# anenbergb/Co-DETR-TensorRT

Hardware: AMD Instinct MI355X
Metric: images/sec, Co-DINO Swin-L 1920x1280 fp16 (p50 ms/image alongside) (higher is better)
Workload: dtype f16

## Files before the change

__graft_entry__.py:

```python
import os
import subprocess
import sys

ROOT = os.path.dirname(os.path.abspath(__file__))
PKG_ROOT = os.path.join(ROOT, "co-detr-tensorrt_amd")
for _p in (ROOT, PKG_ROOT, os.path.join(ROOT, "oracle")):
    if _p not in sys.path:
        sys.path.insert(0, _p)


def _newer(target, sources):
    if not os.path.isfile(target):
        return True
    t = os.path.getmtime(target)
    return any(os.path.getmtime(s) > t for s in sources)


def build() -> None:
    csrc = os.path.join(PKG_ROOT, "csrc")
    so = os.path.join(PKG_ROOT, "codetr", "libcodetr_hip.so")
    srcs = [os.path.join(csrc, f) for f in os.listdir(csrc) if f.endswith((".hip", ".h", "Makefile"))]
    srcs += [os.path.join(ROOT, "include", h) for h in ("codetr_hip.h", "codetr_jpeg.h", "codetr_jpeg_dec.h", "codetr_assign.h", "codetr_wbf.h", "codetr_motion.h", "codetr_appearance.h", "codetr_redact.h")]
    if _newer(so, srcs):
        subprocess.check_call(["make", "-C", csrc, "-s", "-j4"])
    runner_dir = os.path.join(ROOT, "runner")
    runner = os.path.join(runner_dir, "codetr_runner")
    if _newer(runner, [os.path.join(runner_dir, f) for f in ("codetr_runner.cpp", "dispatch_gen.inc", "Makefile")]):
        subprocess.check_call(["make", "-C", runner_dir, "-s"])
    import msda_oracle

    msda_oracle.build()
    import codetr


def smoke() -> None:
    build()
    import smoke_impl

    smoke_impl.run()


if __name__ == "__main__":
    build()
    print("build ok")
    if len(sys.argv) > 1 and sys.argv[1] == "smoke":
        smoke()
        print("smoke ok")
```

co-detr-tensorrt_amd/codetr/_kernel_names.py:

```python
KERNEL_NAMES = (
    "add_kernel",
    "appearance_describe_kernel",
    "assign_kernel",
    "batched_nms_kernel",
    "cast_fp8_kernel",
    "cast_fp8mx_kernel",
    "conv_im2col_nchw_kernel",
    "conv_tokens_kernel",
    "decode_boxes_kernel",
    "decoder_layer_kernel",
    "draw_detections_kernel",
    "encoder_geometry_kernel",
    "ffn_fp8_kernel",
    "ffn_fused_kernel",
    "frames_to_rgb_kernel",
    "gather_rows_kernel",
    "gn_apply_kernel",
    "gn_finalize_kernel",
    "gn_partial_kernel",
    "im2col_tokens_kernel",
    "jpeg_encode_rows_kernel",
    "jpeg_gather_rows_kernel",
    "jpegdec_coefficients",
    "jpegdec_idct",
    "jpegdec_link_runs",
    "jpegdec_pixels",
    "jpegdec_sync_runs",
    "layernorm_fp8_kernel",
    "layernorm_fp8mx_kernel",
    "layernorm_kernel",
    "level_cums_kernel",
    "level_mask_kernel",
    "linear_256_fp8_kernel",
    "linear_256_kernel",
    "linear_kernel",
    "linear_pp_kernel",
    "linear_sk_kernel",
    "linear_xs_kernel",
    "maxpool_tokens_kernel",
    "mha_attention_kernel",
    "motion_finish_kernel",
    "motion_match_kernel",
    "motion_sim_fit_kernel",
    "motion_sim_pairs_kernel",
    "motion_thumb_kernel",
    "msda_backward_generic_kernel",
    "msda_backward_kernel",
    "msda_encoder_v4_kernel",
    "msda_fused_headmajor_kernel",
    "msda_op4_kernel",
    "msda_scalar_kernel",
    "msda_tiled_kernel",
    "pack_w2_kernel",
    "patch_im2col_k4_kernel",
    "postprocess_kernel",
    "postprocess_softnms_kernel",
    "preprocess_batch_kernel",
    "preprocess_kernel",
    "preprocess_tiles_kernel",
    "preprocess_views_kernel",
    "query_sine_embed_kernel",
    "redact_kernel",
    "row_max_kernel",
    "sigmoid_kernel",
    "sine_pos_kernel",
    "slice_merge_kernel",
    "splitk_reduce_kernel",
    "swin_mlp_kernel",
    "topk_kernel",
    "topk_reg_kernel",
    "track_kernel",
    "tta_merge_kernel",
    "valid_ratios_kernel",
    "wbf_merge_kernel",
    "window_attention_kernel",
)
```

co-detr-tensorrt_amd/codetr/export.py:

```python
import ctypes
import struct

import torch

from . import _cabi

MAGIC = b"CODETRPLAN\x00\x02"
import re

from ._kernel_names import KERNEL_NAMES

_OWN_DEMANGLED = re.compile(r"^(?:void )?\(anonymous namespace\)::(" + "|".join(KERNEL_NAMES) + r")\s*[<(]")
_OWN_MANGLED = re.compile(r"^_ZN12_GLOBAL__N_1(\d+)([A-Za-z_][A-Za-z0-9_]*)")


def is_own_kernel(name: str) -> bool:
    if _OWN_DEMANGLED.match(name):
        return True
    m = _OWN_MANGLED.match(name)
    return bool(m) and m.group(2)[:int(m.group(1))] in KERNEL_NAMES
KIND_INT, KIND_FLOAT, KIND_DEV, KIND_NULL, KIND_HOST, KIND_STREAM = 0, 1, 2, 3, 4, 5


def _hip():
    for name in ("libamdhip64.so", "libamdhip64.so.7", "libamdhip64.so.6"):
        try:
            return ctypes.CDLL(name)
        except OSError:
            continue
    raise RuntimeError("libamdhip64.so not found")


def _read_device(hip, addr, nbytes):
    buf = ctypes.create_string_buffer(nbytes)
    rc = hip.hipMemcpy(buf, ctypes.c_void_p(addr), ctypes.c_size_t(nbytes), 2)
    if rc != 0:
        raise RuntimeError(f"hipMemcpy D2H of {nbytes} bytes at {addr:#x} failed with {rc}")
    return buf.raw


def _segments(device):
    segs = []
    for s in torch.cuda.memory_snapshot():
        if s.get("device", 0) != device.index:
            continue
        blocks, addr = [], s["address"]
        for b in s["blocks"]:
            a = b.get("address", addr)
            blocks.append((a, b["size"], b["state"]))
            addr = a + b["size"]
        segs.append({"address": s["address"], "size": s["total_size"], "blocks": blocks})
    return sorted(segs, key=lambda s: s["address"])


@torch.no_grad()
def export_plan(model, batch_inputs, img_masks, path, warmup=2):
    if not batch_inputs.is_cuda or batch_inputs.dtype != torch.float16:
        raise ValueError("export_plan records the fp16 GPU path")
    from . import hip_ops

    ab = hip_ops.nondefault_switches()
    if ab:
        raise RuntimeError(f"export_plan refuses to record under A/B switches: reset {ab}")
    dev = batch_inputs.device
    batch_inputs, img_masks = batch_inputs.contiguous(), img_masks.contiguous()
    hip = _hip()
    hip.hipMemcpy.argtypes = [ctypes.c_void_p, ctypes.c_void_p, ctypes.c_size_t, ctypes.c_int]
    with torch.cuda.device(dev):
        for _ in range(warmup):
            model(batch_inputs, img_masks)
        torch.cuda.synchronize(dev)
        live_before = [(a, n) for s in _segments(dev) for a, n, st in s["blocks"] if st == "active_allocated"]
        initial = [(a, n, _read_device(hip, a, n)) for a, n in live_before]
        _cabi.RECORDER = []
        try:
            with torch.profiler.profile(activities=[torch.profiler.ProfilerActivity.CUDA]) as prof:
                boxes, scores, labels = model(batch_inputs, img_masks)
                torch.cuda.synchronize(dev)
            calls = _cabi.RECORDER
        finally:
            _cabi.RECORDER = None
        foreign = sorted({e.name[:100] for e in prof.events() if e.device_type == torch.autograd.DeviceType.CUDA
                          and not is_own_kernel(e.name)})
        if foreign:
            raise RuntimeError("this model / input shape is not exportable: the forward ran device work outside "
                               f"libcodetr_hip.so that a plan cannot replay: {foreign}")
        want = [t.cpu() for t in (boxes, scores, labels)]
        for t in (boxes, scores, labels):
            t.zero_()
        lib = _cabi.load()
        for name, args in calls:
            rc = getattr(lib, name)(*args)
            if rc:
                raise RuntimeError(f"replay of the recorded launch list failed in {name}: error {rc}")
        torch.cuda.synchronize(dev)
        for what, t, w in zip(("boxes", "scores", "labels"), (boxes, scores, labels), want):
            if not torch.equal(t.cpu(), w):
                raise RuntimeError(f"the recorded launch list does not reproduce the recorded {what}: not exportable")
        segs = _segments(dev)

    def locate(addr, what):
        for i, s in enumerate(segs):
            if s["address"] <= addr < s["address"] + s["size"]:
                return i, addr - s["address"]
        raise RuntimeError(f"{what}: device pointer {addr:#x} is outside every allocator segment")

    used = set()
    enc_calls = []
    for name, args in calls:
        argtypes = _cabi.SIGNATURES[name][1]
        enc = []
        for j, (a, t) in enumerate(zip(args, argtypes)):
            if j == 0:
                enc.append((KIND_STREAM, None))
            elif isinstance(a, (ctypes.Array, ctypes.Structure, ctypes._SimpleCData)) and t is _cabi._vp:
                enc.append((KIND_HOST, bytes(a)))
            elif t is _cabi._vp:
                if a is None or a == 0:
                    enc.append((KIND_NULL, None))
                else:
                    seg, off = locate(int(a), name)
                    used.add(seg)
                    enc.append((KIND_DEV, (seg, off)))
            elif t is ctypes.c_float:
                enc.append((KIND_FLOAT, float(a)))
            else:
                enc.append((KIND_INT, int(a)))
        enc_calls.append((name, enc))

    def io(name, t):
        seg, off = locate(t.data_ptr(), name)
        used.add(seg)
        return (name, seg, off, t.numel() * t.element_size(), str(t.dtype).replace("torch.", ""), tuple(t.shape))

    ios = [io("batch_inputs", batch_inputs), io("img_masks", img_masks), io("boxes", boxes.contiguous()),
           io("scores", scores.contiguous()), io("labels", labels.contiguous())]
    if not (boxes.is_contiguous() and scores.is_contiguous() and labels.is_contiguous()):
        raise RuntimeError("outputs must be contiguous to be addressable by the plan")
    blobs = []
    for a, n, data in initial:
        try:
            seg, off = locate(a, "initial block")
        except RuntimeError:
            continue
        if seg in used:
            blobs.append((seg, off, data))

    with open(path, "wb") as f:
        f.write(MAGIC)
        f.write(struct.pack("<iI", _cabi.ABI_VERSION, len(segs)))
        for i, s in enumerate(segs):
            f.write(struct.pack("<Q", s["size"] if i in used else 0))
        f.write(struct.pack("<I", len(blobs)))
        for seg, off, data in blobs:
            f.write(struct.pack("<IQQ", seg, off, len(data)))
            f.write(data)
        f.write(struct.pack("<I", len(enc_calls)))
        for name, enc in enc_calls:
            nb = name.encode()
            f.write(struct.pack("<H", len(nb)) + nb + struct.pack("<B", len(enc)))
            for kind, v in enc:
                f.write(struct.pack("<B", kind))
                if kind == KIND_INT:
                    f.write(struct.pack("<q", v))
                elif kind == KIND_FLOAT:
                    f.write(struct.pack("<f", v))
                elif kind == KIND_DEV:
                    f.write(struct.pack("<IQ", *v))
                elif kind == KIND_HOST:
                    f.write(struct.pack("<I", len(v)) + v)
        f.write(struct.pack("<I", len(ios)))
        for name, seg, off, nbytes, dtype, shape in ios:
            nb, db = name.encode(), dtype.encode()
            f.write(struct.pack("<H", len(nb)) + nb + struct.pack("<H", len(db)) + db)
            f.write(struct.pack("<IQQB", seg, off, nbytes, len(shape)) + struct.pack(f"<{len(shape)}q", *shape))
    return {"launches": len(enc_calls), "segments": len(segs), "segments_used": len(used),
            "initial_bytes": sum(len(b[2]) for b in blobs), "outputs": {n: s for n, _, _, _, _, s in ios[2:]}}
```

co-detr-tensorrt_amd/codetr/hip_ops.py:

```python

import collections
import math
import os

import numpy as np
import torch
import torch.nn.functional as F

from . import _appearance, _assign, _cabi, _jpeg, _jpeg_dec, _motion, _redact, _wbf

NATIVE = {"msda", "linear(f16/bf16, K%64==0)", "layer_norm(f16/bf16)", "swin_window_attention(f16, head_dim 32)",
          "msda_fused(softmax + sampling locations in-kernel)", "groupnorm_tokens(f16, 8 ch/group)",
          "sine_pos_tokens(f16, + level_embed)", "ffn_fused(f16, 256 -> hidden -> 256, ReLU, + identity)",
          "mask_pyramid(level masks + running valid counts + valid ratios)",
          "query_sine_embed(f16: sigmoid x valid ratios + sine embedding of the decoder reference boxes)",
          "encoder_geometry(f16: reference points, proposals, keep/drop state)", "row_max(f16)",
          "preprocess_image(u8 -> f16/f32, cv2-exact resize + pad + normalise + mask)", "batched_nms(f32)",
          "preprocess_batch(u8 -> f16/bf16/f32, <= 32 images of any size per launch, stacked + padded)",
          "postprocess_detections(f16/bf16/f32: threshold + sort + per-class NMS + rescale, one workgroup per image)",
          "postprocess_detections_soft(f16/bf16/f32: threshold + per-class soft-NMS (linear / naive) + max_per_img + rescale)",
          "patch_merge_layernorm(f16: Swin 2x2 gather + LayerNorm)",
          "msda_encoder_packed(f16/bf16: LDS-staged gather for the encoder's self-attention, csrc/msda_encoder4.hip)",
          "patch_embed(f16/bf16: 4x4 patch gather + GEMM)",
          "mha_attention(f16/bf16: dense softmax attention, head_dim 32, <= 1024 keys)",
          "topk(f16/bf16 rows, k <= 1024: radix select + bitonic sort)",
          "im2col_tokens(16-bit token-major maps)",
          "resnet50(f16/bf16: implicit-GEMM conv_tokens, stem window gather + GEMM, maxpool_tokens, BN folded)",
          "small_ops(f16: add, sigmoid, gather_rows, decode_boxes, valid_ratios)",
          "linear_fp8(e4m3 x e4m3, K%128==0) + layer_norm_fp8 + cast_fp8", "ffn_fp8(fused FFN, both products e4m3)"}


LINEAR_PROFILE = None
KERNEL_PROFILE = None


def _timed(name, meta, launch, device):
    if KERNEL_PROFILE is None:
        return launch()
    st = torch.cuda.current_stream(device)
    e0, e1 = torch.cuda.Event(enable_timing=True), torch.cuda.Event(enable_timing=True)
    e0.record(st)
    r = launch()
    e1.record(st)
    KERNEL_PROFILE.setdefault(name, []).append((e0, e1, meta))
    return r


def _timed_linear(launch, device, M, N, K, *tag):
    if LINEAR_PROFILE is None:
        return launch()
    st = torch.cuda.current_stream(device)
    e0, e1 = torch.cuda.Event(enable_timing=True), torch.cuda.Event(enable_timing=True)
    e0.record(st)
    r = launch()
    e1.record(st)
    if r is not False:
        LINEAR_PROFILE.append((e0, e1, 2.0 * M * N * K, M, N, K) + tag)
    return r


def _gpu(x, what):
    if not x.is_cuda:
        raise RuntimeError(
            f"codetr.hip_ops.{what}: got a {x.device.type} tensor; this package computes on MI355X only "
            "(the CPU formulation is the oracle in oracle/, not a fallback)"
        )


LINEAR_PP = True


def _persistent_ok(mk, head_major, out, x2, w, r2, bias):
    return (mk is None and not head_major and out.data_ptr() % 16 == 0 and x2.data_ptr() % 16 == 0
            and w.data_ptr() % 16 == 0 and (r2 is None or r2.data_ptr() % 16 == 0)
            and (bias is None or bias.data_ptr() % 16 == 0))


def linear(x, weight, bias=None, act=None, residual=None, row_mask=None, head_major=None):
    _gpu(x, "linear")
    if _cabi.linear_supported(x, weight):
        K = x.shape[-1]
        N = weight.shape[0]
        x2 = x.reshape(-1, K)
        if not x2.is_contiguous():
            x2 = x2.contiguous()
        w = weight if weight.is_contiguous() else weight.contiguous()
        r2 = None
        if residual is not None:
            r2 = residual.reshape(-1, N)
            if not r2.is_contiguous():
                r2 = r2.contiguous()
        mk = None
        if row_mask is not None:
            mk = row_mask.reshape(-1)
            if mk.dtype != torch.bool and mk.dtype != torch.uint8:
                mk = mk != 0
            mk = mk.contiguous()
        hm_rows = hm_hd = 0
        if head_major:
            if x.dim() != 3 or residual is not None:
                raise ValueError("head_major needs a [B, S, K] input and no residual")
            hm_rows, hm_hd = x.shape[1], int(head_major)
        out = torch.empty((x2.shape[0], N), dtype=x.dtype, device=x.device)
        if x2.shape[0] > 0:
            with torch.cuda.device(x.device):
                res_act = act == "relu_res"
                splits, ws_bytes = (1, 0) if (head_major or res_act) else _cabi.linear_splitk_plan(x2.shape[0], N, K)
                if res_act:
                    launch = lambda: _cabi.linear(x2, w, bias, r2, act, out, mk, hm_rows, hm_hd)
                elif splits > 1:
                    ws = torch.empty(ws_bytes, dtype=torch.uint8, device=x.device)
                    launch = lambda: _cabi.linear_splitk(x2, w, bias, r2, act, out, splits, ws, mk)
                elif (LINEAR_PP and _persistent_ok(mk, head_major, out, x2, w, r2, bias)
                      and _cabi.linear_pp_preferred(x2.shape[0], N, K, act, r2 is not None)):
                    launch = lambda: _cabi.linear_pp(x2, w, bias, r2, act, out)
                elif (_persistent_ok(mk, head_major, out, x2, w, r2, bias)
                      and _cabi.linear_sk_preferred(x2.shape[0], N, K, act, r2 is not None)):
                    launch = lambda: _cabi.linear_sk(x2, w, bias, r2, act, out)
                else:
                    launch = lambda: _cabi.linear(x2, w, bias, r2, act, out, mk, hm_rows, hm_hd)
                _timed_linear(launch, x.device, x2.shape[0], N, K)
        if head_major:
            return out.view(x.shape[0], N // hm_hd, hm_rows, hm_hd)
        return out.view(*x.shape[:-1], N)
    if head_major:
        raise RuntimeError("head_major output exists only on the native linear (f16/bf16, K % 64 == 0)")
    y = F.linear(x, weight, bias)
    if act == "relu_res":
        if row_mask is not None:
            y = y.masked_fill(row_mask[..., None], 0.0)
        return F.relu(y + residual if residual is not None else y)
    if act == "relu":
        y = F.relu(y, inplace=True)
    elif act == "gelu":
        y = F.gelu(y)
    elif act is not None:
        raise ValueError(act)
    if row_mask is not None:
        y = y.masked_fill(row_mask[..., None], 0.0)
    if residual is not None:
        y = y + residual
    return y


LN_GEMM = True


def linear_ln_supported(x, norm_weight, weight):
    return (LN_GEMM and x.is_cuda and norm_weight is not None and norm_weight.dtype == x.dtype and weight.dtype == x.dtype
            and not torch.is_grad_enabled() and norm_weight.shape[0] == x.shape[-1]
            and _cabi.linear_xadd_supported(x.numel() // max(x.shape[-1], 1), weight.shape[0], x.shape[-1], x.dtype))


def linear_ln(x, norm_weight, norm_bias, eps, weight, bias=None, act=None):
    _gpu(x, "linear_ln")
    if linear_ln_supported(x, norm_weight, weight):
        K, N = x.shape[-1], weight.shape[0]
        x2 = x.reshape(-1, K)
        x2 = x2 if x2.is_contiguous() else x2.contiguous()
        w = weight if weight.is_contiguous() else weight.contiguous()
        out = torch.empty((x2.shape[0], N), dtype=x.dtype, device=x.device)
        with torch.cuda.device(x.device):
            ok = _timed_linear(lambda: _cabi.linear_ln(x2, norm_weight, norm_bias, eps, w, bias, act, out),
                               x.device, x2.shape[0], N, K)
        if ok:
            return out.view(*x.shape[:-1], N)
    return linear(layer_norm(x, norm_weight, norm_bias, eps), weight, bias, act=act)


XADD = True
XADD_MIN_ROWS = 0


def linear_xadd_supported(x, x_add, weight):
    return (XADD and x.is_cuda and x_add is not None and x_add.shape == x.shape and x_add.dtype == x.dtype
            and weight.dtype == x.dtype and not torch.is_grad_enabled()
            and x.numel() // max(x.shape[-1], 1) >= XADD_MIN_ROWS
            and _cabi.linear_xadd_supported(x.numel() // max(x.shape[-1], 1), weight.shape[0], x.shape[-1], x.dtype))


def linear_xadd(x, x_add, weight, bias=None):
    _gpu(x, "linear_xadd")
    if linear_xadd_supported(x, x_add, weight):
        K, N = x.shape[-1], weight.shape[0]
        x2, a2 = x.reshape(-1, K), x_add.reshape(-1, K)
        x2 = x2 if x2.is_contiguous() else x2.contiguous()
        a2 = a2 if a2.is_contiguous() else a2.contiguous()
        w = weight if weight.is_contiguous() else weight.contiguous()
        out = torch.empty((x2.shape[0], N), dtype=x.dtype, device=x.device)
        with torch.cuda.device(x.device):
            ok = _timed_linear(lambda: _cabi.linear_xadd(x2, a2, w, bias, out), x.device, x2.shape[0], N, K)
        if ok:
            return out.view(*x.shape[:-1], N)
    return linear(x + x_add, weight, bias)


FFN_FUSED_MIN_ROWS = 24576


def ffn_fused_supported(x, w1, w2, act):
    return (x.is_cuda and x.numel() // max(x.shape[-1], 1) >= FFN_FUSED_MIN_ROWS
            and _cabi.ffn_fused_supported(x, w1, w2, act))


def derived(params, name, build):
    first = params[0]
    key = tuple((id(p), p.data_ptr(), p._version, p.dtype, p.device) for p in params)
    hit = getattr(first, name, None)
    if hit is not None and hit[0] == key:
        return hit[1]
    with torch.no_grad():
        val = build()
    setattr(first, name, (key, val))
    return val


def _packed_w2(w2):
    hit = getattr(w2, "_codetr_packed_w2", None)
    if hit is None or hit[0] != w2._version or hit[1].device != w2.device or hit[1].dtype != w2.dtype:
        with torch.no_grad(), torch.cuda.device(w2.device):
            hit = (w2._version, _cabi.ffn_pack_w2(w2.detach().contiguous()))
        w2._codetr_packed_w2 = hit
    return hit[1]


SWIN_MLP = True
SWIN_MLP_MIN_ROWS = 32768


def swin_mlp_supported(x, ln_weight, w1, w2, act):
    C = x.shape[-1]
    return (SWIN_MLP and x.is_cuda and x.dtype in (torch.float16, torch.bfloat16) and act == "gelu" and C in (192, 384)
            and w1.shape == (4 * C, C) and w2.shape == (C, 4 * C) and ln_weight is not None
            and x.numel() // C >= SWIN_MLP_MIN_ROWS and w1.dtype == x.dtype and w2.dtype == x.dtype)


def swin_mlp(x, ln_weight, ln_bias, eps, w1, b1, w2, b2):
    _gpu(x, "swin_mlp")
    C = x.shape[-1]
    x2 = x.reshape(-1, C)
    if not x2.is_contiguous():
        x2 = x2.contiguous()
    out = torch.empty_like(x2)
    w1c = w1 if w1.is_contiguous() else w1.contiguous()
    with torch.cuda.device(x.device):
        w2p = _packed_w2(w2)
        _timed("swin_mlp", {"M": x2.shape[0], "C": C},
               lambda: _cabi.swin_mlp(x2, ln_weight, ln_bias, eps, w1c, b1, w2p, b2, out), x.device)
    return out.view(x.shape)


def ffn_fused(x, w1, b1, w2, b2, ln=None, pos=None, ln_in=None):
    _gpu(x, "ffn_fused")
    x2 = x.reshape(-1, x.shape[-1])
    if not x2.is_contiguous():
        x2 = x2.contiguous()
    out = torch.empty_like(x2)
    p2 = out2 = None
    if pos is not None:
        p2 = pos.reshape(-1, pos.shape[-1])
        if p2.shape != x2.shape or p2.dtype != x2.dtype:
            raise ValueError("pos must match x in shape and dtype")
        if not p2.is_contiguous():
            p2 = p2.contiguous()
        out2 = torch.empty_like(x2)
    if x2.shape[0] > 0:
        with torch.cuda.device(x.device):
            _timed("ffn_fused", {"M": x2.shape[0], "C": x2.shape[1], "hidden": w1.shape[0]},
                   lambda: _cabi.ffn_fused(x2, w1.contiguous(), b1, _packed_w2(w2), b2, out, ln, p2, out2, ln_in), x.device)
    if pos is not None:
        return out.view(x.shape), out2.view(x.shape)
    return out.view(x.shape)


FFN_OPROJ = True


def ffn_oproj_fused(attn, wo, bo, identity, w1, b1, w2, b2, ln, pos=None, ln_in=None):
    _gpu(attn, "ffn_oproj_fused")
    C = attn.shape[-1]
    a2, i2 = attn.reshape(-1, C), identity.reshape(-1, C)
    a2 = a2 if a2.is_contiguous() else a2.contiguous()
    i2 = i2 if i2.is_contiguous() else i2.contiguous()
    if i2.shape != a2.shape or i2.dtype != a2.dtype:
        raise ValueError("identity must match the attention output in shape and dtype")
    out = torch.empty_like(a2)
    p2 = out2 = None
    if pos is not None:
        p2 = pos.reshape(-1, C)
        if p2.shape != a2.shape or p2.dtype != a2.dtype:
            raise ValueError("pos must match x in shape and dtype")
        p2 = p2 if p2.is_contiguous() else p2.contiguous()
        out2 = torch.empty_like(a2)
    w1p = derived((w1,), "_codetr_w1_oproj", lambda: w1.detach()[:, torch.tensor(
        _cabi.ffn_oproj_w1_index(C), dtype=torch.long, device=w1.device)].contiguous())
    woc = wo if wo.is_contiguous() else wo.contiguous()
    if a2.shape[0] > 0:
        with torch.cuda.device(attn.device):
            _timed("ffn_fused", {"M": a2.shape[0], "C": C, "hidden": w1.shape[0], "oproj": True},
                   lambda: _cabi.ffn_oproj_fused(a2, woc, bo, i2, w1p, b1, _packed_w2(w2), b2, out, ln_in, ln, p2, out2),
                   attn.device)
    if pos is not None:
        return out.view(attn.shape), out2.view(attn.shape)
    return out.view(attn.shape)


def layer_norm(x, weight, bias, eps=1e-5):
    _gpu(x, "layer_norm")
    if _cabi.layernorm_supported(x, weight):
        C = x.shape[-1]
        x2 = x.reshape(-1, C)
        if not x2.is_contiguous():
            x2 = x2.contiguous()
        out = torch.empty_like(x2)
        if x2.shape[0] > 0:
            with torch.cuda.device(x.device):
                _cabi.layernorm(x2, weight, bias, eps, out)
        return out.view(x.shape)
    return F.layer_norm(x, (x.shape[-1],), weight, bias, eps)


MERGE_LN = True


def patch_merge_layernorm_supported(x, C):
    return (x.is_cuda and x.dtype in (torch.float16, torch.bfloat16) and C % 8 == 0 and 4 * C <= 4096
            and MERGE_LN)


def patch_merge_layernorm(x, hw, weight_kkc, bias_kkc, eps=1e-5):
    _gpu(x, "patch_merge_layernorm")
    B, L, C = x.shape
    H, W = hw
    x4 = x.view(B, H, W, C)
    if not x4.is_contiguous():
        x4 = x4.contiguous()
    with torch.cuda.device(x.device):
        return _cabi.patch_merge_layernorm(x4, weight_kkc, bias_kkc, eps)


def group_norm(x, groups, weight, bias, eps=1e-5):
    _gpu(x, "group_norm")
    return F.group_norm(x, groups, weight, bias, eps)


def groupnorm_tokens_supported(x, groups):
    return x.is_cuda and _cabi.groupnorm_tokens_supported(x, groups)


def groupnorm_tokens_into(x, gamma, beta, groups, eps, dest, row_start):
    _gpu(x, "groupnorm_tokens_into")
    B, HW, C = x.shape
    if not x.is_contiguous():
        x = x.contiguous()
    if not dest.is_contiguous() or dest.shape[0] != B or dest.shape[2] != C:
        raise AssertionError("destination must be a contiguous [B, S, C] tensor")
    with torch.cuda.device(x.device):
        _cabi.groupnorm_tokens(x, gamma, beta, groups, eps, dest[0, row_start:], dest.shape[1] * C)
    return dest


def query_sine_embed_supported(ref, valid_ratios, pos_feat):
    return (ref.is_cuda and ref.dtype in (torch.float16, torch.bfloat16) and valid_ratios.dtype == ref.dtype
            and ref.shape[-1] in (2, 4) and pos_feat % 8 == 0 and valid_ratios.shape[1] <= ref.shape[-1] * pos_feat // 8)


def query_sine_embed(ref, valid_ratios, pos_feat, temperature=10000.0):
    _gpu(ref, "query_sine_embed")
    vr32 = getattr(valid_ratios, "_codetr_f32", None) if MSDA_FP32_REF else None
    with torch.cuda.device(ref.device):
        ref_in, embed, ref32 = _cabi.query_sine_embed(ref.contiguous(), valid_ratios.contiguous(), pos_feat, temperature,
                                                      valid_ratios32=vr32)
    if ref32 is not None:
        ref_in._codetr_ref32 = ref32
    return ref_in, embed


def encoder_geometry(valid_ratios, mask_flat, shapes):
    _gpu(mask_flat, "encoder_geometry")
    if valid_ratios.dtype not in (torch.float16, torch.bfloat16):
        raise RuntimeError("encoder_geometry is the 16-bit inference path; fp32 parity runs use the ATen formulation")
    with torch.cuda.device(mask_flat.device):
        return _cabi.encoder_geometry(valid_ratios.contiguous(), mask_flat.contiguous(),
                                      [tuple(int(v) for v in s) for s in shapes])


def row_max(x):
    _gpu(x, "row_max")
    if x.dtype not in (torch.float16, torch.bfloat16) or not x.is_contiguous():
        return x.max(-1)[0]
    with torch.cuda.device(x.device):
        return _cabi.row_max(x.view(-1, x.shape[-1])).view(x.shape[:-1])


def preprocess_image(src_u8, resized_hw, pad_hw, mean, std, pad_value=(0, 0, 0), dtype=torch.float16):
    _gpu(src_u8, "preprocess_image")
    if src_u8.dtype != torch.uint8 or src_u8.dim() != 3 or src_u8.shape[2] != 3:
        raise ValueError("expected a uint8 [H, W, 3] image")
    with torch.cuda.device(src_u8.device):
        return _cabi.preprocess_u8(src_u8.contiguous(), resized_hw, pad_hw, mean, std, pad_value, dtype)


def batched_nms(boxes, scores, labels, iou_threshold):
    _gpu(boxes, "batched_nms")
    if boxes.shape[0] == 0:
        return torch.empty((0,), dtype=torch.int64, device=boxes.device)
    order = torch.sort(scores.float(), descending=True, stable=True)[1]
    with torch.cuda.device(boxes.device):
        keep = _cabi.batched_nms_sorted(boxes.float()[order].contiguous(), labels.to(torch.int64)[order].contiguous(),
                                        iou_threshold)
    return order[keep]


PREPROCESS_BATCH_MAX = _cabi.PREPROCESS_BATCH_MAX


def _preprocess_rows(name, launch, src_u8, rows, batch_hw, mean, std, pad_val, pad_value, dtype, with_mask):
    _gpu(src_u8, name)
    if src_u8.dtype != torch.uint8 or src_u8.dim() != 1 or not src_u8.is_contiguous():
        raise ValueError("expected one contiguous flat uint8 buffer")
    if dtype not in (torch.float16, torch.bfloat16, torch.float32):
        raise ValueError(f"{name} writes f16, bf16 or f32, not {dtype}")
    N = len(rows)
    H, W = (int(v) for v in batch_hw)
    x = torch.empty((N, 3, H, W), dtype=dtype, device=src_u8.device)
    m = torch.empty((N, H, W), dtype=dtype, device=src_u8.device) if with_mask else None
    with torch.cuda.device(src_u8.device):
        for i in range(0, N, PREPROCESS_BATCH_MAX):
            j = min(N, i + PREPROCESS_BATCH_MAX)
            launch(src_u8, rows[i:j], (H, W), mean, std, pad_val, pad_value, x[i:j], m[i:j] if m is not None else None)
    return x, m


def preprocess_batch(src_u8, images, batch_hw, mean, std, pad_val=(0, 0, 0), pad_value=0.0, dtype=torch.float16,
                     with_mask=True):
    return _preprocess_rows("preprocess_batch", _cabi.preprocess_batch_u8, src_u8, images, batch_hw, mean, std, pad_val,
                            pad_value, dtype, with_mask)


def preprocess_views(src_u8, rows8, batch_hw, mean, std, pad_val=(0, 0, 0), pad_value=0.0, dtype=torch.float16,
                     with_mask=True):
    if any(len(r) != 8 for r in rows8):
        raise ValueError("preprocess_views: eight values per row, the last one the flip (0 or 1)")
    return _preprocess_rows("preprocess_views", _cabi.preprocess_views_u8, src_u8, rows8, batch_hw, mean, std, pad_val,
                            pad_value, dtype, with_mask)


def preprocess_tiles(src_u8, rows11, batch_hw, mean, std, pad_val=(0, 0, 0), pad_value=0.0, dtype=torch.float16,
                     with_mask=True):
    if any(len(r) != 11 for r in rows11):
        raise ValueError("preprocess_tiles: eleven values per row (src_offset, H_img, W_img, y0, x0, H_crop, W_crop, "
                         "H_resized, W_resized, H_pad, W_pad)")
    return _preprocess_rows("preprocess_tiles", _cabi.preprocess_tiles_u8, src_u8, rows11, batch_hw, mean, std, pad_val,
                            pad_value, dtype, with_mask)


Detections = collections.namedtuple("Detections", "boxes scores labels count packed")
SoftDetections = collections.namedtuple("SoftDetections", "boxes scores labels count index packed")


def _detection_views(packed, N, Q, dtype, with_index):
    es = torch.empty((), dtype=dtype).element_size()
    o1 = N * Q * 8
    o2 = o1 + N * 4
    o3 = o2 + (N * Q * 4 if with_index else 0)
    o4 = o3 + N * Q * 4 * es
    o5 = o4 + N * Q * es
    boxes, scores = packed[o3:o4].view(dtype).view(N, Q, 4), packed[o4:o5].view(dtype).view(N, Q)
    labels, count = packed[:o1].view(torch.int64).view(N, Q), packed[o1:o2].view(torch.int32)
    if not with_index:
# ... 955 lines not shown
    if state.device != src_u8.device:
        raise ValueError("estimate_motion: the state lives on another device than the images")
    rows = [tuple(int(v) for v in r) for r in rows]
    N = len(rows)
    for off, H, W in rows:
        if not (1 <= H <= _cabi.FRAME_MAX_SIDE and 1 <= W <= _cabi.FRAME_MAX_SIDE) or off < 0 or off + H * W * 3 > src_u8.numel():
            raise ValueError(f"estimate_motion: image (offset {off}, {H}x{W}) outside the buffer or larger than "
                             f"{_cabi.FRAME_MAX_SIDE} a side")
    streams = track_streams(streams, N)
    if any(v >= state.shape[0] for v in streams):
        raise ValueError(f"estimate_motion: a stream index outside the state's {state.shape[0]} streams")
    motion = torch.empty((N, 8 if sim else 4), dtype=torch.float32, device=src_u8.device)
    diag = torch.empty((N, 8 if sim else 4), dtype=torch.int32, device=src_u8.device)
    four = (cfg["grid"], cfg["search"], cfg["texture"], cfg["min_blocks"])
    with torch.cuda.device(src_u8.device):
        for i in range(0, N, PREPROCESS_BATCH_MAX):
            j = min(N, i + PREPROCESS_BATCH_MAX)
            nbytes = _motion.work2_bytes(j - i) if sim else _motion.work_bytes(j - i)
            work = torch.empty((nbytes,), dtype=torch.uint8, device=src_u8.device)
            if sim:
                _motion.estimate(src_u8, rows[i:j], streams[i:j], state, four, work, motion[i:j], diag[i:j], similarity=True)
            else:
                _motion.estimate(src_u8, rows[i:j], streams[i:j], state, four, work, motion[i:j], diag[i:j])
    return motion, diag


ASSIGN_MAX_ROWS, ASSIGN_MAX_COLS, ASSIGN_MAX_GAIN = _assign.MAX_ROWS, _assign.MAX_COLS, _assign.MAX_GAIN


def linear_assignment(gain):
    if not torch.is_tensor(gain) or gain.dtype != torch.int32 or gain.dim() not in (2, 3):
        raise ValueError("linear_assignment: gain must be an int32 tensor [n, m] or [B, n, m]")
    B, n, m = gain.shape if gain.dim() == 3 else (1,) + tuple(gain.shape)
    if n > ASSIGN_MAX_ROWS or m > ASSIGN_MAX_COLS:
        raise ValueError(f"linear_assignment: at most {ASSIGN_MAX_ROWS} rows x {ASSIGN_MAX_COLS} columns, got {n} x {m}")
    _gpu(gain, "linear_assignment")
    g = gain.contiguous().view(B, n, m)
    match = torch.full((B, n), -1, dtype=torch.int32, device=g.device)
    total = torch.zeros((B,), dtype=torch.int64, device=g.device)
    if B and n and m:
        with torch.cuda.device(g.device):
            for i in range(0, B, 65535):
                _assign.assign(g[i:i + 65535], match[i:i + 65535], total[i:i + 65535])
    return (match, total) if gain.dim() == 3 else (match[0], total[0])


def track_streams(streams, N):
    def one(v):
        if isinstance(v, bool) or not isinstance(v, (int, np.integer)) or v < 0:
            raise ValueError(f"streams: non-negative integers, got {v!r}")
        return int(v)

    if streams is None:
        return [0] * N
    if isinstance(streams, (int, np.integer)):
        return [one(streams)] * N
    if not isinstance(streams, (list, tuple, np.ndarray)) or len(streams) != N:
        raise ValueError(f"streams: one non-negative integer, or one per frame ({N})")
    return [one(v) for v in streams]


def mask_pyramid(img_masks, shapes):
    _gpu(img_masks, "mask_pyramid")
    m = img_masks
    if m.dtype not in (torch.bool, torch.uint8, torch.float16, torch.bfloat16, torch.float32):
        m = m != 0
    with torch.cuda.device(m.device):
        return _cabi.mask_pyramid(m.contiguous(), [tuple(int(v) for v in s) for s in shapes])


def level_cums(ycum, xcum, B, start, hw):
    n = hw[0] * hw[1]
    return (ycum[B * start:B * (start + n)].view(B, hw[0], hw[1]), xcum[B * start:B * (start + n)].view(B, hw[0], hw[1]))


def sine_pos_tokens_into(mask, dest, row_start, level_embed, num_feats, temperature, scale, eps, offset, normalize,
                         cums=None):
    if cums is None:
        _gpu(mask, "sine_pos_tokens_into")
        valid = ~mask
        ycum = valid.cumsum(1, dtype=torch.float32).contiguous()
        xcum = valid.cumsum(2, dtype=torch.float32).contiguous()
    else:
        ycum, xcum = cums
        _gpu(ycum, "sine_pos_tokens_into")
    if dest.dtype not in (torch.float16, torch.bfloat16) or not dest.is_contiguous() or dest.shape[2] != 2 * num_feats:
        raise AssertionError("destination must be a contiguous f16 / bf16 [B, S, 2*num_feats] tensor")
    if level_embed is not None and level_embed.dtype != dest.dtype:
        level_embed = level_embed.to(dest.dtype)
    with torch.cuda.device(ycum.device):
        _cabi.sine_pos_tokens(ycum, xcum, level_embed, dest[0, row_start:], dest.shape[1] * dest.shape[2], num_feats,
                              temperature, scale, eps, offset, normalize)
    return dest


def conv2d(x, weight, bias=None, stride=1, padding=0):
    _gpu(x, "conv2d")
    return F.conv2d(x, weight, bias, stride=stride, padding=padding)


def window_attention(qkv, rel_bias, mask, num_heads):
    _gpu(qkv, "window_attention")
    nWB, N, C3 = qkv.shape
    C = C3 // 3
    hd = C // num_heads
    qkv = qkv.view(nWB, N, 3, num_heads, hd).permute(2, 0, 3, 1, 4)
    q, k, v = qkv[0], qkv[1], qkv[2]
    attn = (q * hd ** -0.5) @ k.transpose(-2, -1)
    attn = attn + rel_bias.unsqueeze(0)
    if mask is not None:
        nW = mask.shape[0]
        attn = (attn.view(nWB // nW, nW, num_heads, N, N) + mask[None, :, None]).view(nWB, num_heads, N, N)
    attn = attn.softmax(-1)
    return (attn @ v).transpose(1, 2).reshape(nWB, N, C)


def swin_window_attention_supported(x, embed_dims, num_heads, window_size):
    return x.is_cuda and _cabi.window_attention_supported(x.dtype, embed_dims, num_heads, window_size)


WINDOW_BIAS_LANE = True
_LANE_INDEX = {}


def _rel_bias_lane_order(rel_bias, window_size):
    if window_size not in _LANE_INDEX:
        _LANE_INDEX[window_size] = _cabi.window_attention_bias_index(window_size)
    idx = _LANE_INDEX[window_size]
    if idx is None:
        return None
    return derived((rel_bias,), "_codetr_rel_bias_lane",
                   lambda: rel_bias[..., torch.tensor(idx, dtype=torch.long, device=rel_bias.device)].contiguous())


def swin_window_attention(qkv, qkv_bias, rel_bias, hw_shape, num_heads, window_size, shift, out_scale=None, out_mx=False):
    _gpu(qkv, "swin_window_attention")
    B, L, C3 = qkv.shape
    H, W = hw_shape
    if L != H * W:
        raise AssertionError("input feature has wrong size")
    if not qkv.is_contiguous():
        qkv = qkv.contiguous()
    if qkv_bias is None:
        qkv_bias = torch.zeros(C3, dtype=qkv.dtype, device=qkv.device)
    if (out_scale is not None or out_mx) and qkv.dtype != torch.float16:
        raise ValueError("the e4m3 output forms take fp16 qkv")
    out = torch.empty((B, L, C3 // 3), dtype=FP8 if (out_scale is not None or out_mx) else qkv.dtype, device=qkv.device)
    scales = torch.empty(_cabi.mx_scale_bytes(B * L, C3 // 3), dtype=torch.uint8, device=qkv.device) if out_mx else None
    rel_bias = rel_bias.contiguous()
    lane = _rel_bias_lane_order(rel_bias, window_size) if WINDOW_BIAS_LANE else None
    with torch.cuda.device(qkv.device):
        _timed("window_attention", {"rows": B * L, "C": C3 // 3, "heads": num_heads, "window": window_size,
                                    "out_bytes": out.element_size()},
               lambda: _cabi.window_attention(qkv, qkv_bias, rel_bias if lane is None else lane, out, B, H, W, num_heads,
                                              window_size, shift, out_scale, scales, 0 if lane is None else 1), qkv.device)
    return (out, scales) if out_mx else out


def mha_self_attention(q, k, v, num_heads):
    _gpu(q, "mha_self_attention")
    B, N, C = q.shape
    if _cabi.mha_attention_supported(q, k, v, num_heads):
        out = torch.empty((B, N, C), dtype=q.dtype, device=q.device)
        with torch.cuda.device(q.device):
            _cabi.mha_attention(q, k, v, num_heads, out)
        return out
    hd = C // num_heads
    sp = lambda t: t.reshape(B, -1, num_heads, hd).transpose(1, 2)
    o = F.scaled_dot_product_attention(sp(q), sp(k), sp(v))
    return o.transpose(1, 2).reshape(B, N, C)


def msda_fused_supported(value_dtype, head_dim, num_levels, num_points):
    return _cabi.msda_fused_supported(value_dtype, head_dim, num_levels, num_points)


def msda_head_major_supported(value_dtype, head_dim, num_levels, num_points):
    return _cabi.msda_head_major_supported(value_dtype, head_dim, num_levels, num_points)


def msda_fused(value, spatial_shapes, level_start_index, proj, off_col, logit_col, reference_points, num_levels,
               num_points, head_major=False):
    _gpu(value, "msda_fused")
    if head_major:
        B, M, S, D = value.shape
    else:
        B, S, M, D = value.shape
    out = torch.empty((B, proj.shape[1], M * D), dtype=value.dtype, device=value.device)
    ref32 = getattr(reference_points, "_codetr_ref32", None) if MSDA_FP32_REF else None
    ref = ref32 if ref32 is not None else reference_points.to(value.dtype).contiguous()
    if out.numel():
        with torch.cuda.device(value.device):
            _timed("msda_fused", {"B": B, "S": S, "Nq": proj.shape[1], "M": M, "D": D, "L": num_levels, "P": num_points},
                   lambda: _cabi.msda_fused(value.contiguous(), spatial_shapes, level_start_index, proj.contiguous(),
                                            off_col, logit_col, ref, num_levels, num_points, out,
                                            head_major=head_major), value.device)
    return out


def patch_embed_supported(x, weight, stride):
    kh, kw = weight.shape[-2:]
    return (x.is_cuda and x.dtype in (torch.float16, torch.bfloat16) and weight.dtype == x.dtype
            and kh == kw == 4 and tuple(stride) == (4, 4) and x.shape[1] * 16 <= 64 and not torch.is_grad_enabled())


def patch_embed(x, weight, bias):
    _gpu(x, "patch_embed")
    B, C, H, W = x.shape
    E = weight.shape[0]
    Hp, Wp = -(-H // 4), -(-W // 4)
    cache = getattr(weight, "_codetr_w64", None)
    if cache is None or cache[0] != weight._version or cache[1].device != weight.device:
        w64 = torch.zeros((E, 64), dtype=weight.dtype, device=weight.device)
        w64[:, :C * 16] = weight.detach().reshape(E, C * 16)
        cache = weight._codetr_w64 = (weight._version, w64)
    cols = torch.empty((B * Hp * Wp, 64), dtype=x.dtype, device=x.device)
    with torch.cuda.device(x.device):
        _cabi.patch_im2col(x.contiguous(), 4, 64, cols)
    return linear(cols, cache[1], bias).view(B, Hp * Wp, E), (Hp, Wp)


def im2col_tokens(x4d, k, stride, pad):
    _gpu(x4d, "im2col_tokens")
    B, H, W, C = x4d.shape
    Ho, Wo = (H + 2 * pad - k) // stride + 1, (W + 2 * pad - k) // stride + 1
    if x4d.dtype in (torch.float16, torch.bfloat16) and C % 8 == 0:
        out = torch.empty((B, Ho * Wo, k * k * C), dtype=x4d.dtype, device=x4d.device)
        with torch.cuda.device(x4d.device):
            _cabi.im2col_tokens(x4d.contiguous(), k, stride, pad, out)
        return out
    xp = F.pad(x4d, (0, 0, pad, pad, pad, pad))
    return torch.cat([xp[:, ky:ky + stride * (Ho - 1) + 1:stride, kx:kx + stride * (Wo - 1) + 1:stride, :]
                      for ky in range(k) for kx in range(k)], dim=-1).reshape(B, Ho * Wo, -1)


R50_NATIVE = True
R50_CONV_IM2COL = False


def conv_tokens(x4d, weight_kkc, bias, k, stride, pad, act=None, residual=None):
    _gpu(x4d, "conv_tokens")
    B, H, W, C = x4d.shape
    Cout = weight_kkc.shape[0]
    Ho, Wo = (H + 2 * pad - k) // stride + 1, (W + 2 * pad - k) // stride + 1
    if not _cabi.conv_tokens_supported(x4d, weight_kkc, k, stride, pad):
        raise RuntimeError(f"conv_tokens: no native kernel for x {tuple(x4d.shape)} {x4d.dtype}, k={k}, stride={stride}, "
                           f"pad={pad}, Cout={Cout} (C % 64 == 0, Cout % 8 == 0, k in (1, 3), stride in (1, 2))")
    if R50_CONV_IM2COL:
        cols = im2col_tokens(x4d, k, stride, pad)
        r = residual.reshape(B, Ho * Wo, Cout) if residual is not None else None
        return linear(cols, weight_kkc, bias, act=act, residual=r).view(B, Ho, Wo, Cout)
    x4d = x4d if x4d.is_contiguous() else x4d.contiguous()
    if residual is not None and not residual.is_contiguous():
        residual = residual.contiguous()
    out = torch.empty((B, Ho, Wo, Cout), dtype=x4d.dtype, device=x4d.device)
    with torch.cuda.device(x4d.device):
        _timed("conv_tokens", {"M": B * Ho * Wo, "N": Cout, "K": k * k * C},
               lambda: _cabi.conv_tokens(x4d, weight_kkc, bias, residual, k, stride, pad, act, out), x4d.device)
    return out


def stem_conv_tokens(x, weight_pad, bias, k, stride, pad):
    _gpu(x, "stem_conv_tokens")
    B, C, H, W = x.shape
    Cout, kpad = weight_pad.shape
    Ho, Wo = (H + 2 * pad - k) // stride + 1, (W + 2 * pad - k) // stride + 1
    cols = torch.empty((B * Ho * Wo, kpad), dtype=x.dtype, device=x.device)
    with torch.cuda.device(x.device):
        _cabi.conv_im2col_nchw(x if x.is_contiguous() else x.contiguous(), k, stride, pad, kpad, cols)
    return linear(cols, weight_pad, bias, act="relu").view(B, Ho, Wo, Cout)


def maxpool_tokens(x4d):
    _gpu(x4d, "maxpool_tokens")
    B, H, W, C = x4d.shape
    out = torch.empty((B, (H - 1) // 2 + 1, (W - 1) // 2 + 1, C), dtype=x4d.dtype, device=x4d.device)
    with torch.cuda.device(x4d.device):
        _cabi.maxpool_tokens(x4d if x4d.is_contiguous() else x4d.contiguous(), out)
    return out




def topk(x, k, want_values=True):
    _gpu(x, "topk")
    x2 = x.reshape(-1, x.shape[-1])
    if not torch.is_grad_enabled():
        x2 = x2 if x2.is_contiguous() else x2.contiguous()
        if _cabi.topk_supported(x2, k):
            idx = torch.empty((x2.shape[0], k), dtype=torch.int64, device=x.device)
            val = torch.empty((x2.shape[0], k), dtype=x.dtype, device=x.device) if want_values else None
            with torch.cuda.device(x.device):
                _cabi.topk(x2, k, val, idx)
            shape = (*x.shape[:-1], k)
            return (val.view(shape) if val is not None else None), idx.view(shape)
    v, i = torch.topk(x, k, dim=-1)
    return v, i


MSDA_ENCODER = True
MSDA_FP32_REF = True


_SWITCH_DEFAULTS = {"ENC_POSGEN": True, "WINDOW_BIAS_LANE": True, "LINEAR_PP": True, "SWIN_MLP": True, "SWIN_MLP_MIN_ROWS": 32768, "LN_GEMM": True, "XADD": True, "XADD_MIN_ROWS": 0, "MERGE_LN": True, "MSDA_ENCODER": True,
                    "MSDA_FP32_REF": True, "FP8_MIN_TILES": 96,
                    "R50_NATIVE": True, "R50_CONV_IM2COL": False}


def nondefault_switches():
    import sys

    from . import multi_scale_deformable_attention as msda_mod
    from . import transformer as tr_mod

    me = sys.modules[__name__]
    out = [k for k, v in _SWITCH_DEFAULTS.items() if getattr(me, k) != v]
    if msda_mod.HEAD_MAJOR_VALUE:
        out.append("HEAD_MAJOR_VALUE")
    out += [k for k in ("DEC_FUSED", "DEC_VPROJ") if not getattr(tr_mod, k)]
    return sorted(out)


MSDA_V4 = True
MSDA_V4_THREADS = 512
MSDA_V4_REGION = (16, 16)
MSDA_V4_LDS_BUDGET = 64 * 1024
MSDA_V4_MARGIN_CAP = 40.0
MSDA_V4_HEAD_MAJOR = True
ENC_PROJ_FUSED = True
_SWITCH_DEFAULTS.update({"MSDA_V4": True, "MSDA_V4_THREADS": 512, "MSDA_V4_REGION": (16, 16),
                         "MSDA_V4_LDS_BUDGET": 64 * 1024, "MSDA_V4_MARGIN_CAP": 40.0,
                         "MSDA_V4_HEAD_MAJOR": True, "ENC_PROJ_FUSED": True, "FFN_OPROJ": True})


def msda_encoder_packed_supported(dtype, head_dim, num_levels, num_points):
    return (MSDA_V4 and MSDA_ENCODER and dtype in (torch.float16, torch.bfloat16) and head_dim == 32 and num_levels == 5
            and num_points == 4)


def value_projection_f16(x, weight, bias, row_mask, head_dim):
    _gpu(x, "value_projection_f16")
    if not (x.dtype == torch.bfloat16 and weight.dtype == torch.bfloat16 and x.dim() == 3):
        return None
    B, S, K = x.shape
    N = weight.shape[0]
    x2 = x.reshape(-1, K)
    x2 = x2 if x2.is_contiguous() else x2.contiguous()
    w = weight if weight.is_contiguous() else weight.contiguous()
    mk = None
    if row_mask is not None:
        mk = row_mask.reshape(-1)
        if mk.dtype != torch.bool and mk.dtype != torch.uint8:
            mk = mk != 0
        mk = mk.contiguous()
    out = torch.empty((B * S, N), dtype=torch.float16, device=x.device)
    with torch.cuda.device(x.device):
        ok = _cabi.linear_bf16_f16out(x2, w, bias, out, mk, S, int(head_dim))
    return out.view(B, N // head_dim, S, head_dim) if ok else None


ENC_POSGEN = True


def encoder_projections(x, pos, w_cat, b_cat, row_mask, n_value, head_dim):
    _gpu(x, "encoder_projections")
    if not (ENC_PROJ_FUSED and x.dim() == 3 and x.dtype in (torch.float16, torch.bfloat16) and pos is not None
            and pos.shape == x.shape and pos.dtype == x.dtype and w_cat.dtype == x.dtype and not torch.is_grad_enabled()):
        return None
    B, S, K = x.shape
    n_packed = w_cat.shape[0] - n_value
    x2, p2 = x.reshape(-1, K), pos.reshape(-1, K)
    x2 = x2 if x2.is_contiguous() else x2.contiguous()
    p2 = p2 if p2.is_contiguous() else p2.contiguous()
    mk = None
    if row_mask is not None:
        mk = row_mask.reshape(-1)
        if mk.dtype != torch.bool and mk.dtype != torch.uint8:
            mk = mk != 0
        mk = mk.contiguous()
    value = torch.empty((B * S, n_value), dtype=torch.float16, device=x.device)
    packed = torch.empty((B * S, n_packed), dtype=x.dtype, device=x.device)
    gen = getattr(pos, "_codetr_posgen", None) if ENC_POSGEN else None

    def launch():
        if gen is not None and gen["S"] == S and gen["B"] == B:
            if _cabi.encoder_projections_posgen(x2, S, gen["cums"], gen["shapes"], gen["level_embed"], gen["temperature"],
                                                gen["scale"], gen["eps"], gen["offset"], gen["normalize"], w_cat, b_cat,
                                                mk, value, packed, S, int(head_dim)):
                return True
        return _cabi.encoder_projections(x2, p2, w_cat, b_cat, mk, value, packed, S, int(head_dim))

    with torch.cuda.device(x.device):
        ok = _timed_linear(launch, x.device, B * S, n_value + n_packed, K)
    if not ok:
        return None
    return value.view(B, n_value // head_dim, S, head_dim), packed.view(B, S, n_packed)


def msda_packed_projection(w_off, b_off, w_aw, b_aw, num_heads, num_levels, num_points):
    idx = _cabi.msda_pack_projection_index(num_heads, num_levels, num_points)
    if idx is None:
        return None
    ii = torch.tensor(idx, dtype=torch.long, device=w_off.device)
    wcat = torch.cat((w_off, w_aw), 0)
    bcat = torch.cat((b_off, b_aw), 0)
    pad = ii < 0
    wp = wcat[ii.clamp_min(0)].clone()
    bp = bcat[ii.clamp_min(0)].clone()
    wp[pad] = 0
    bp[pad] = 0
    return wp.contiguous(), bp.contiguous()


def msda_encoder_windows_packed(bias, level_shapes, num_heads, num_levels, num_points):
    import math

    b = bias.detach().float().cpu().view(num_heads, num_levels, num_points, 2)
    b = torch.round(b * 1024) / 1024
    lo, hi = b.amin(2).tolist(), b.amax(2).tolist()
    groups = [[0], [1, 2], [3, 4]]
    steps = int(2 * MSDA_V4_MARGIN_CAP)

    def window(m, l, mg):
        return (max(-127, math.floor(lo[m][l][0] - mg)), min(127, math.ceil(hi[m][l][0] + mg)),
                max(-127, math.floor(lo[m][l][1] - mg)), min(127, math.ceil(hi[m][l][1] + mg)))

    def need(trial):
        return _cabi.msda_encoder_packed_lds_bytes(level_shapes, num_heads, num_points, [trial] * num_heads,
                                                   MSDA_V4_REGION, MSDA_V4_THREADS)

    out = []
    for m in range(num_heads):
        win = [window(m, l, 0.0) for l in range(num_levels)]
        for grp in groups:
            a, z = 0, steps
            while a < z:
                mid = (a + z + 1) // 2
                trial = list(win)
                for l in grp:
                    trial[l] = window(m, l, 0.5 * mid)
                n = need(trial)
                if 0 < n <= MSDA_V4_LDS_BUDGET:
                    a = mid
                else:
                    z = mid - 1
            for l in grp:
                win[l] = window(m, l, 0.5 * a)
        out.append(win)
    return out


def msda_encoder_packed(value, level_shapes, packed, num_points, windows, valid_counts, head_major=False):
    _gpu(value, "msda_encoder_packed")
    if head_major:
        B, M, S, D = value.shape
    else:
        B, S, M, D = value.shape
    if not (valid_counts is not None and valid_counts.dtype == torch.float32 and valid_counts.is_contiguous()
            and valid_counts.shape == (B, len(level_shapes), 2) and packed.shape[:2] == (B, S) and packed.is_contiguous()):
        return None
    if value.dtype != torch.float16 or packed.dtype not in (torch.float16, torch.bfloat16):
        return None
    out = torch.empty((B, S, M * D), dtype=packed.dtype, device=value.device)
    ok = [True]

    def run():
        ok[0] = _cabi.msda_encoder_packed(value.contiguous(), level_shapes, packed, num_points, windows, valid_counts,
                                          MSDA_V4_REGION, MSDA_V4_THREADS, out, head_major)

    with torch.cuda.device(value.device):
        _timed("msda_fused", {"B": B, "S": S, "Nq": S, "M": M, "D": D, "L": len(level_shapes), "P": num_points},
               run, value.device)
    return out if ok[0] else None


def msda(value, spatial_shapes, level_start_index, sampling_locations, attention_weights, im2col_step):
    return torch.ops.codetr.multi_scale_deformable_attention(
        value, spatial_shapes, level_start_index, sampling_locations, attention_weights, im2col_step
    )


FP8 = _cabi.FP8
FP8_MAX = 448.0
FP8_MIN_TILES = 96


def fp8_weight(weight):
    def build():
        w = weight.detach().float()
        scale = (w.abs().amax(1) / FP8_MAX).clamp_min(1e-12)
        return (w / scale[:, None]).to(FP8).contiguous(), scale.contiguous()

    return derived((weight,), "_codetr_fp8_w", build)


def ffn_fp8_supported(x, w1, w2, act):
    return (ffn_fused_supported(x, w1, w2, act) and x.dtype == torch.float16 and w1.shape[0] % 128 == 0
            and w1.shape[0] <= 2048)


def ffn_fp8_weights(w1, w2):
    def build():
        a, b = w1.detach().float(), w2.detach().float()
        s1 = (a.abs().amax(1) / FP8_MAX).clamp_min(1e-12)
        s2 = (b.abs().amax(1) / FP8_MAX).clamp_min(1e-12)
        p = torch.arange(128, device=w2.device)
        g, t, r = p // 32, (p % 32) // 4, p % 4
        src = 16 * t + 4 * g + r
        bq = (b / s2[:, None]).to(FP8).view(torch.uint8).view(b.shape[0], -1, 128)[:, :, src].reshape(b.shape).contiguous()
        return (a / s1[:, None]).to(FP8).contiguous(), s1.contiguous(), bq.view(FP8), s2.contiguous()

    return derived((w1, w2), "_codetr_ffn_fp8_w", build)


def ffn_fp8(x, w1, b1, w2, b2, x_scale, h_scale, ln=None, pos=None, ln_in=None):
    _gpu(x, "ffn_fp8")
    x2 = x.reshape(-1, x.shape[-1])
    if not x2.is_contiguous():
        x2 = x2.contiguous()
    out = torch.empty_like(x2)
    p2 = out2 = None
    if pos is not None:
        p2 = pos.reshape(-1, pos.shape[-1])
        if p2.shape != x2.shape or p2.dtype != x2.dtype:
            raise ValueError("pos must match x in shape and dtype")
        if not p2.is_contiguous():
            p2 = p2.contiguous()
        out2 = torch.empty_like(x2)
    w1q, s1, w2q, s2 = ffn_fp8_weights(w1, w2)
    if x2.shape[0] > 0:
        with torch.cuda.device(x.device):
            _timed("ffn_fp8", {"M": x2.shape[0], "C": x2.shape[1], "hidden": w1.shape[0]},
                   lambda: _cabi.ffn_fp8(x2, w1q, s1, b1, w2q, s2, b2, out, x_scale, h_scale, ln, p2, out2, ln_in), x.device)
    if pos is not None:
        return out.view(x.shape), out2.view(x.shape)
    return out.view(x.shape)


def linear_fp8_supported(rows, weight):
    N, K = weight.shape
    return (weight.is_cuda and weight.dtype == torch.float16 and K % 128 == 0 and N % 8 == 0
            and -(-rows // 256) * -(-N // 256) >= FP8_MIN_TILES
            and rows * N <= 0x7fffffff)


def linear_fp8(x8, x_scale, weight, bias=None, act=None, residual=None, out_scale=None):
    _gpu(x8, "linear_fp8")
    w8, ws = fp8_weight(weight)
    K, N = x8.shape[-1], weight.shape[0]
    x2 = x8.reshape(-1, K)
    r2 = None if residual is None else residual.reshape(-1, N).contiguous()
    out = torch.empty((x2.shape[0], N), dtype=FP8 if out_scale is not None else torch.float16, device=x8.device)
    with torch.cuda.device(x8.device):
        launch = lambda: _cabi.linear_fp8(x2, w8, ws, x_scale, bias, r2, act, out, out_scale or 0.0)
        _timed_linear(launch, x8.device, x2.shape[0], N, K, "fp8")
    return out.view(*x8.shape[:-1], N)


def linear_fp8mx(x8, x_scales, weight, bias=None, act=None, residual=None, out_mx=False):
    _gpu(x8, "linear_fp8mx")
    w8, ws = fp8_weight(weight)
    K, N = x8.shape[-1], weight.shape[0]
    x2 = x8.reshape(-1, K)
    r2 = None if residual is None else residual.reshape(-1, N).contiguous()
    out = torch.empty((x2.shape[0], N), dtype=FP8 if out_mx else torch.float16, device=x8.device)
    sy = torch.empty(_cabi.mx_scale_bytes(x2.shape[0], N), dtype=torch.uint8, device=x8.device) if out_mx else None
    with torch.cuda.device(x8.device):
        launch = lambda: _cabi.linear_fp8mx(x2, x_scales, w8, ws, bias, r2, act, out, sy)
        _timed_linear(launch, x8.device, x2.shape[0], N, K, "fp8")
    out = out.view(*x8.shape[:-1], N)
    return (out, sy) if out_mx else out


def cast_fp8mx(x):
    _gpu(x, "cast_fp8mx")
    x2 = x.reshape(-1, x.shape[-1])
    x2 = x2 if x2.is_contiguous() else x2.contiguous()
    out = torch.empty(x2.shape, dtype=FP8, device=x.device)
    sy = torch.empty(_cabi.mx_scale_bytes(*x2.shape), dtype=torch.uint8, device=x.device)
    with torch.cuda.device(x.device):
        _cabi.cast_fp8mx(x2, out, sy)
    return out.view(x.shape), sy


def layer_norm_fp8mx(x, weight, bias, eps):
    _gpu(x, "layer_norm_fp8mx")
    C = x.shape[-1]
    x2 = x.reshape(-1, C)
    x2 = x2 if x2.is_contiguous() else x2.contiguous()
    out = torch.empty(x2.shape, dtype=FP8, device=x.device)
    sy = torch.empty(_cabi.mx_scale_bytes(x2.shape[0], C), dtype=torch.uint8, device=x.device)
    with torch.cuda.device(x.device):
        _cabi.layernorm_fp8mx(x2, weight, bias, eps, out, sy)
    return out.view(x.shape), sy


def mx_dequant(x8, scales):
    x2 = x8.reshape(-1, x8.shape[-1])
    M, K = x2.shape
    m = torch.arange(M, device=x8.device)[:, None]
    kb = torch.arange(K // 32, device=x8.device)[None, :]
    MB = -(-M // 128)
    idx = ((((kb >> 2) * MB + (m >> 7)) * 64 + (kb & 3) * 16 + (m & 15)) * 8 + ((m >> 4) & 7)).long()
    e = scales.long()[idx].float() - 127.0
    return (x2.float().view(M, K // 32, 32) * torch.exp2(e)[:, :, None]).view(x8.shape)


# ... 89 lines not shown
```

co-detr-tensorrt_amd/codetr/swin.py:

```python
import warnings
from collections import OrderedDict

import torch
import torch.nn as nn
import torch.nn.functional as F

from . import hip_ops
from .transformer_layers import FFN, build_norm


def to_2tuple(x):
    return tuple(x) if isinstance(x, (tuple, list)) else (x, x)


class PatchEmbed(nn.Module):

    def __init__(self, in_channels=3, embed_dims=768, conv_type="Conv2d", kernel_size=16, stride=16, padding="corner",
                 dilation=1, bias=True, norm_cfg=None, input_size=None, init_cfg=None):
        super().__init__()
        if padding != "corner" or dilation != 1:
            raise NotImplementedError("PatchEmbed: only 'corner' padding, dilation 1 (what Swin uses)")
        self.embed_dims = embed_dims
        self.kernel_size, self.stride = to_2tuple(kernel_size), to_2tuple(stride or kernel_size)
        self.projection = nn.Conv2d(in_channels, embed_dims, self.kernel_size, self.stride, bias=bias)
        self.norm = build_norm(norm_cfg, embed_dims) if norm_cfg is not None else None

    def forward(self, x):
        H, W = x.shape[-2:]
        kh, kw = self.kernel_size
        sh, sw = self.stride
        if hip_ops.patch_embed_supported(x, self.projection.weight, self.stride):
            x, hw = hip_ops.patch_embed(x, self.projection.weight, self.projection.bias)
            if self.norm is not None:
                x = hip_ops.layer_norm(x, self.norm.weight, self.norm.bias, self.norm.eps)
            return x, hw
        ph = max((-(-H // sh) - 1) * sh + kh - H, 0)
        pw = max((-(-W // sw) - 1) * sw + kw - W, 0)
        if ph or pw:
            x = F.pad(x, (0, pw, 0, ph))
        x = hip_ops.conv2d(x, self.projection.weight, self.projection.bias, stride=self.stride)
        hw = (x.shape[2], x.shape[3])
        x = x.flatten(2).transpose(1, 2)
        if self.norm is not None:
            x = hip_ops.layer_norm(x, self.norm.weight, self.norm.bias, self.norm.eps)
        return x, hw


class PatchMerging(nn.Module):

    def __init__(self, in_channels, out_channels, kernel_size=2, stride=None, padding="corner", dilation=1, bias=False,
                 norm_cfg=dict(type="LN"), init_cfg=None):
        super().__init__()
        if to_2tuple(kernel_size) != (2, 2) or to_2tuple(stride or kernel_size) != (2, 2) or padding != "corner":
            raise NotImplementedError("PatchMerging: only the 2x2 / stride-2 / corner-padded form Swin uses")
        self.in_channels, self.out_channels = in_channels, out_channels
        self.norm = build_norm(norm_cfg, 4 * in_channels) if norm_cfg is not None else None
        self.reduction = nn.Linear(4 * in_channels, out_channels, bias=bias)

    def forward(self, x, input_size):
        B, L, C = x.shape
        H, W = input_size
        if L != H * W:
            raise AssertionError("input feature has wrong size")
        x = x.view(B, H, W, C)
        if H % 2 or W % 2:
            x = F.pad(x, (0, 0, 0, W % 2, 0, H % 2))
        H2, W2 = (H + 1) // 2, (W + 1) // 2
        if x.is_cuda and not torch.is_grad_enabled():
            nw, nb, rw = self._permuted_params(C)
            if (self.norm is not None and isinstance(self.norm, nn.LayerNorm)
                    and hip_ops.patch_merge_layernorm_supported(x, C)):
                x = hip_ops.patch_merge_layernorm(x.reshape(B, -1, C), (2 * H2, 2 * W2), nw, nb, self.norm.eps)
                return hip_ops.linear(x, rw, self.reduction.bias), (H2, W2)
            x = x.view(B, H2, 2, W2, 2, C).permute(0, 1, 3, 2, 4, 5).reshape(B, H2 * W2, 4 * C)
            if self.norm is not None:
                x = hip_ops.layer_norm(x, nw, nb, self.norm.eps)
            return hip_ops.linear(x, rw, self.reduction.bias), (H2, W2)
        x = x.view(B, H2, 2, W2, 2, C).permute(0, 1, 3, 5, 2, 4).reshape(B, H2 * W2, 4 * C)
        if self.norm is not None:
            x = hip_ops.layer_norm(x, self.norm.weight, self.norm.bias, self.norm.eps)
        return hip_ops.linear(x, self.reduction.weight, self.reduction.bias), (H2, W2)

    def _permuted_params(self, C):
        ps = [self.reduction.weight] + ([self.norm.weight, self.norm.bias] if self.norm is not None else [])

        def build():
            idx = (torch.arange(C, device=ps[0].device)[None, :] * 4 + torch.arange(4, device=ps[0].device)[:, None]).reshape(-1)
            rw = self.reduction.weight.detach()[:, idx].contiguous()
            nw = self.norm.weight.detach()[idx].contiguous() if self.norm is not None else None
            nb = self.norm.bias.detach()[idx].contiguous() if self.norm is not None else None
            return nw, nb, rw

        return hip_ops.derived(ps, "_codetr_perm", build)


class WindowMSA(nn.Module):
    def __init__(self, embed_dims, num_heads, window_size, qkv_bias=True, qk_scale=None, attn_drop_rate=0.0,
                 proj_drop_rate=0.0, init_cfg=None):
        super().__init__()
        self.embed_dims, self.window_size, self.num_heads = embed_dims, to_2tuple(window_size), num_heads
        head_dim = embed_dims // num_heads
        if qk_scale is not None and qk_scale != head_dim ** -0.5:
            raise NotImplementedError("custom qk_scale")
        self.scale = head_dim ** -0.5
        Wh, Ww = self.window_size
        self.relative_position_bias_table = nn.Parameter(torch.zeros((2 * Wh - 1) * (2 * Ww - 1), num_heads))
        coords = torch.stack(torch.meshgrid(torch.arange(Wh), torch.arange(Ww), indexing="ij")).flatten(1)
        rel = coords[:, :, None] - coords[:, None, :]
        index = (rel[0] + Wh - 1) * (2 * Ww - 1) + (rel[1] + Ww - 1)
        self.register_buffer("relative_position_index", index.contiguous())
        self.qkv = nn.Linear(embed_dims, embed_dims * 3, bias=qkv_bias)
        self.proj = nn.Linear(embed_dims, embed_dims)

    def init_weights(self):
        nn.init.trunc_normal_(self.relative_position_bias_table, std=0.02)

    def relative_position_bias(self):
        t = self.relative_position_bias_table
        N = self.window_size[0] * self.window_size[1]
        return hip_ops.derived((t,), "_codetr_rel_bias", lambda: t[self.relative_position_index.view(-1)].view(N, N, -1)
                               .permute(2, 0, 1).contiguous().detach())

    def forward(self, x, mask=None):
        qkv = hip_ops.linear(x, self.qkv.weight, self.qkv.bias)
        o = hip_ops.window_attention(qkv, self.relative_position_bias(), mask, self.num_heads)
        return hip_ops.linear(o, self.proj.weight, self.proj.bias)


_MASK_CACHE = {}


def shifted_window_mask(Hp, Wp, ws, shift, dtype, device):
    key = (Hp, Wp, ws, shift, dtype, str(device))
    m = _MASK_CACHE.get(key)
    if m is None:
        region = torch.zeros(Hp, Wp, dtype=torch.float32)
        cnt = 0
        for hs in (slice(0, -ws), slice(-ws, -shift), slice(-shift, None)):
            for wsl in (slice(0, -ws), slice(-ws, -shift), slice(-shift, None)):
                region[hs, wsl] = cnt
                cnt += 1
        r = region.view(Hp // ws, ws, Wp // ws, ws).permute(0, 2, 1, 3).reshape(-1, ws * ws)
        diff = r[:, None, :] - r[:, :, None]
        m = torch.where(diff != 0, torch.tensor(-100.0), torch.tensor(0.0)).to(device=device, dtype=dtype)
        _MASK_CACHE[key] = m
    return m


class ShiftWindowMSA(nn.Module):
    def __init__(self, embed_dims, num_heads, window_size, shift_size=0, qkv_bias=True, qk_scale=None,
                 attn_drop_rate=0, proj_drop_rate=0, dropout_layer=dict(type="DropPath", drop_prob=0.0), init_cfg=None):
        super().__init__()
        self.window_size, self.shift_size = window_size, shift_size
        if not 0 <= shift_size < window_size:
            raise AssertionError("shift_size must be in [0, window_size)")
        self.w_msa = WindowMSA(embed_dims, num_heads, to_2tuple(window_size), qkv_bias, qk_scale, attn_drop_rate,
                               proj_drop_rate)

    def takes_norm(self, query, hw_shape):
        return hip_ops.swin_window_attention_supported(query, self.w_msa.embed_dims, self.w_msa.num_heads, self.window_size)

    def forward(self, query, hw_shape, identity=None, pre_norm=None):
        B, L, C = query.shape
        H, W = hw_shape
        if L != H * W:
            raise AssertionError("input feature has wrong size")
        ws, sh = self.window_size, self.shift_size
        m = self.w_msa
        if hip_ops.swin_window_attention_supported(query, C, m.num_heads, ws):
            if pre_norm is not None:
                qkv = hip_ops.linear_ln(query, pre_norm[0], pre_norm[1], pre_norm[2], m.qkv.weight, m.qkv.bias)
            else:
                qkv = hip_ops.linear(query, m.qkv.weight, m.qkv.bias)
            o = hip_ops.swin_window_attention(qkv, m.qkv.bias, m.relative_position_bias(), hw_shape, m.num_heads, ws, sh)
            return hip_ops.linear(o, m.proj.weight, m.proj.bias, residual=identity)
        x = query.view(B, H, W, C)
        pad_r, pad_b = (-W) % ws, (-H) % ws
        if pad_r or pad_b:
            x = F.pad(x, (0, 0, 0, pad_r, 0, pad_b))
        Hp, Wp = H + pad_b, W + pad_r
        mask = None
        if sh > 0:
            x = torch.roll(x, shifts=(-sh, -sh), dims=(1, 2))
            mask = shifted_window_mask(Hp, Wp, ws, sh, query.dtype, query.device)
        win = x.view(B, Hp // ws, ws, Wp // ws, ws, C).permute(0, 1, 3, 2, 4, 5).reshape(-1, ws * ws, C)
        win = self.w_msa(win, mask)
        x = win.view(B, Hp // ws, Wp // ws, ws, ws, C).permute(0, 1, 3, 2, 4, 5).reshape(B, Hp, Wp, C)
        if sh > 0:
            x = torch.roll(x, shifts=(sh, sh), dims=(1, 2))
        if pad_r or pad_b:
            x = x[:, :H, :W, :]
        x = x.reshape(B, H * W, C)
        return x if identity is None else x + identity


class SwinBlock(nn.Module):
    def __init__(self, embed_dims, num_heads, feedforward_channels, window_size=7, shift=False, qkv_bias=True,
                 qk_scale=None, drop_rate=0.0, attn_drop_rate=0.0, drop_path_rate=0.0, act_cfg=dict(type="GELU"),
                 norm_cfg=dict(type="LN"), with_cp=False, init_cfg=None):
        super().__init__()
        self.norm1 = build_norm(norm_cfg, embed_dims)
        self.attn = ShiftWindowMSA(embed_dims, num_heads, window_size, window_size // 2 if shift else 0, qkv_bias,
                                   qk_scale, attn_drop_rate, drop_rate)
        self.norm2 = build_norm(norm_cfg, embed_dims)
        self.ffn = FFN(embed_dims=embed_dims, feedforward_channels=feedforward_channels, num_fcs=2, ffn_drop=drop_rate,
                       act_cfg=act_cfg, add_identity=True)

    def forward(self, x, hw_shape):
        n1, n2 = self.norm1, self.norm2
        mode = getattr(self, "fp8_mode", None)
        if mode is not None and x.is_cuda and x.dtype == torch.float16 and self.attn.takes_norm(x, hw_shape):
            rows = x.shape[0] * x.shape[1]
            if mode == "calibrate":
                return self._forward_fp8_calibrate(x, hw_shape)
            if mode == "run" and all(hip_ops.linear_fp8_supported(rows, w) for w in self._fp8_weights()):
                return self._forward_fp8(x, hw_shape)
            if mode == "mx":
                ops = getattr(self, "fp8_ops", None) or ("qkv", "proj", "fc1", "fc2")
                ws = dict(zip(("qkv", "proj", "fc1", "fc2"), self._fp8_weights()))
                if ops and all(hip_ops.linear_fp8_supported(rows, ws[o]) for o in ops):
                    return self._forward_fp8mx(x, hw_shape)
        if (isinstance(n1, nn.LayerNorm) and self.attn.takes_norm(x, hw_shape)
                and hip_ops.linear_ln_supported(x, n1.weight, self.attn.w_msa.qkv.weight)):
            x = self.attn(x, hw_shape, identity=x, pre_norm=(n1.weight, n1.bias, n1.eps))
        else:
            h = hip_ops.layer_norm(x, n1.weight, n1.bias, n1.eps)
            x = self.attn(h, hw_shape, identity=x)
        fc1, fc2 = self.ffn.layers[0][0], self.ffn.layers[1]
        if (isinstance(n2, nn.LayerNorm) and self.ffn.add_identity and fc1.bias is not None and fc2.bias is not None
                and hip_ops.swin_mlp_supported(x, n2.weight, fc1.weight, fc2.weight, self.ffn.act)):
            return hip_ops.swin_mlp(x, n2.weight, n2.bias, n2.eps, fc1.weight, fc1.bias, fc2.weight, fc2.bias)
        if (isinstance(n2, nn.LayerNorm) and self.ffn.add_identity
                and hip_ops.linear_ln_supported(x, n2.weight, fc1.weight)):
            h = hip_ops.linear_ln(x, n2.weight, n2.bias, n2.eps, fc1.weight, fc1.bias, act=self.ffn.act)
            return hip_ops.linear(h, fc2.weight, fc2.bias, residual=x)
        h = hip_ops.layer_norm(x, n2.weight, n2.bias, n2.eps)
        return self.ffn(h, identity=x)


    def _fp8_weights(self):
        m = self.attn.w_msa
        return (m.qkv.weight, m.proj.weight, self.ffn.layers[0][0].weight, self.ffn.layers[1].weight)

    def _forward_fp8_calibrate(self, x, hw_shape):
        n1, n2, m = self.norm1, self.norm2, self.attn.w_msa
        fc1, fc2 = self.ffn.layers[0][0], self.ffn.layers[1]
        amax = self.__dict__.setdefault("_fp8_amax", {})

        def rec(key, t):
            v = t.detach().abs().amax().float()
            amax[key] = v if key not in amax else torch.maximum(amax[key], v)

        h = hip_ops.layer_norm(x, n1.weight, n1.bias, n1.eps)
        rec("ln1", h)
        qkv = hip_ops.linear(h, m.qkv.weight, m.qkv.bias)
        o = hip_ops.swin_window_attention(qkv, m.qkv.bias, m.relative_position_bias(), hw_shape, m.num_heads,
                                          self.attn.window_size, self.attn.shift_size)
        rec("attn", o)
        x = hip_ops.linear(o, m.proj.weight, m.proj.bias, residual=x)
        h = hip_ops.layer_norm(x, n2.weight, n2.bias, n2.eps)
        rec("ln2", h)
        g = hip_ops.linear(h, fc1.weight, fc1.bias, act=self.ffn.act)
        rec("act", g)
        return hip_ops.linear(g, fc2.weight, fc2.bias, residual=x)

    def _forward_fp8(self, x, hw_shape):
        n1, n2, m = self.norm1, self.norm2, self.attn.w_msa
        fc1, fc2 = self.ffn.layers[0][0], self.ffn.layers[1]
        sc = self._fp8_scales
        h8 = hip_ops.layer_norm_fp8(x, n1.weight, n1.bias, n1.eps, sc["ln1"])
        qkv = hip_ops.linear_fp8(h8, sc["ln1"], m.qkv.weight, m.qkv.bias)
        o8 = hip_ops.swin_window_attention(qkv, m.qkv.bias, m.relative_position_bias(), hw_shape, m.num_heads,
                                           self.attn.window_size, self.attn.shift_size, out_scale=sc["attn"])
        x = hip_ops.linear_fp8(o8, sc["attn"], m.proj.weight, m.proj.bias, residual=x)
        h8 = hip_ops.layer_norm_fp8(x, n2.weight, n2.bias, n2.eps, sc["ln2"])
        g8 = hip_ops.linear_fp8(h8, sc["ln2"], fc1.weight, fc1.bias, act=self.ffn.act, out_scale=sc["act"])
        return hip_ops.linear_fp8(g8, sc["act"], fc2.weight, fc2.bias, residual=x)


    def _forward_fp8mx(self, x, hw_shape):
        n1, n2, m = self.norm1, self.norm2, self.attn.w_msa
        fc1, fc2 = self.ffn.layers[0][0], self.ffn.layers[1]
        ops = getattr(self, "fp8_ops", None) or ("qkv", "proj", "fc1", "fc2")
        if "qkv" in ops:
            h8, hs = hip_ops.layer_norm_fp8mx(x, n1.weight, n1.bias, n1.eps)
            qkv = hip_ops.linear_fp8mx(h8, hs, m.qkv.weight, m.qkv.bias)
        elif hip_ops.linear_ln_supported(x, n1.weight, m.qkv.weight):
            qkv = hip_ops.linear_ln(x, n1.weight, n1.bias, n1.eps, m.qkv.weight, m.qkv.bias)
        else:
            qkv = hip_ops.linear(hip_ops.layer_norm(x, n1.weight, n1.bias, n1.eps), m.qkv.weight, m.qkv.bias)
        if "proj" in ops:
            o8, os_ = hip_ops.swin_window_attention(qkv, m.qkv.bias, m.relative_position_bias(), hw_shape, m.num_heads,
                                                    self.attn.window_size, self.attn.shift_size, out_mx=True)
            x = hip_ops.linear_fp8mx(o8, os_, m.proj.weight, m.proj.bias, residual=x)
        else:
            o = hip_ops.swin_window_attention(qkv, m.qkv.bias, m.relative_position_bias(), hw_shape, m.num_heads,
                                              self.attn.window_size, self.attn.shift_size)
            x = hip_ops.linear(o, m.proj.weight, m.proj.bias, residual=x)
        if "fc1" in ops:
            h8, hs = hip_ops.layer_norm_fp8mx(x, n2.weight, n2.bias, n2.eps)
            if "fc2" in ops:
                g8, gs = hip_ops.linear_fp8mx(h8, hs, fc1.weight, fc1.bias, act=self.ffn.act, out_mx=True)
            else:
                g = hip_ops.linear_fp8mx(h8, hs, fc1.weight, fc1.bias, act=self.ffn.act)
        else:
            if hip_ops.linear_ln_supported(x, n2.weight, fc1.weight):
                g = hip_ops.linear_ln(x, n2.weight, n2.bias, n2.eps, fc1.weight, fc1.bias, act=self.ffn.act)
            else:
                g = hip_ops.linear(hip_ops.layer_norm(x, n2.weight, n2.bias, n2.eps), fc1.weight, fc1.bias, act=self.ffn.act)
            if "fc2" in ops:
                g8, gs = hip_ops.cast_fp8mx(g)
        if "fc2" in ops:
            return hip_ops.linear_fp8mx(g8, gs, fc2.weight, fc2.bias, residual=x)
        return hip_ops.linear(g, fc2.weight, fc2.bias, residual=x)


class SwinBlockSequence(nn.Module):
    def __init__(self, embed_dims, num_heads, feedforward_channels, depth, window_size=7, qkv_bias=True, qk_scale=None,
                 drop_rate=0.0, attn_drop_rate=0.0, drop_path_rate=0.0, downsample=None, act_cfg=dict(type="GELU"),
                 norm_cfg=dict(type="LN"), with_cp=False, init_cfg=None):
        super().__init__()
        self.blocks = nn.ModuleList(
            SwinBlock(embed_dims, num_heads, feedforward_channels, window_size, shift=bool(i % 2), qkv_bias=qkv_bias,
                      qk_scale=qk_scale, drop_rate=drop_rate, attn_drop_rate=attn_drop_rate, act_cfg=act_cfg,
                      norm_cfg=norm_cfg) for i in range(depth))
        self.downsample = downsample

    def forward(self, x, hw_shape):
        for blk in self.blocks:
            x = blk(x, hw_shape)
        if self.downsample is not None:
            x_down, down_hw = self.downsample(x, hw_shape)
            return x_down, down_hw, x, hw_shape
        return x, hw_shape, x, hw_shape


class SwinTransformer(nn.Module):
    def __init__(self, pretrain_img_size=224, in_channels=3, embed_dims=96, patch_size=4, window_size=7, mlp_ratio=4,
                 depths=(2, 2, 6, 2), num_heads=(3, 6, 12, 24), strides=(4, 2, 2, 2), out_indices=(0, 1, 2, 3),
                 qkv_bias=True, qk_scale=None, patch_norm=True, drop_rate=0.0, attn_drop_rate=0.0, drop_path_rate=0.1,
                 use_abs_pos_embed=False, act_cfg=dict(type="GELU"), norm_cfg=dict(type="LN"), with_cp=False,
                 pretrained=None, convert_weights=False, frozen_stages=-1, init_cfg=None):
        super().__init__()
        if init_cfg and pretrained:
            raise AssertionError("init_cfg and pretrained cannot be specified at the same time")
        if isinstance(pretrained, str):
            warnings.warn('DeprecationWarning: pretrained is deprecated, please use "init_cfg" instead')
            init_cfg = dict(type="Pretrained", checkpoint=pretrained)
        elif pretrained is not None:
            raise TypeError("pretrained must be a str or None")
        if use_abs_pos_embed:
            raise NotImplementedError("absolute position embedding is not used by the Co-DETR configs")
        self.init_cfg, self.convert_weights, self.frozen_stages = init_cfg, convert_weights, frozen_stages
        self.out_indices = tuple(out_indices)
        if strides[0] != patch_size:
            raise AssertionError("Use non-overlapping patch embed.")
        self.patch_embed = PatchEmbed(in_channels, embed_dims, "Conv2d", patch_size, strides[0],
                                      norm_cfg=norm_cfg if patch_norm else None)
        self.drop_after_pos = nn.Dropout(p=drop_rate)
        self.stages = nn.ModuleList()
        C = embed_dims
        n = len(depths)
        for i in range(n):
            down = PatchMerging(C, 2 * C, stride=strides[i + 1], norm_cfg=norm_cfg if patch_norm else None) \
                if i < n - 1 else None
            self.stages.append(SwinBlockSequence(C, num_heads[i], mlp_ratio * C, depths[i], window_size, qkv_bias,
                                                 qk_scale, drop_rate, attn_drop_rate, 0.0, down, act_cfg, norm_cfg))
            if down is not None:
                C = down.out_channels
        self.num_features = [int(embed_dims * 2 ** i) for i in range(n)]
        for i in self.out_indices:
            self.add_module(f"norm{i}", build_norm(norm_cfg, self.num_features[i]))

    def init_weights(self):
        for m in self.modules():
            if isinstance(m, nn.Linear):
                nn.init.trunc_normal_(m.weight, std=0.02)
                if m.bias is not None:
                    nn.init.zeros_(m.bias)
            elif isinstance(m, nn.LayerNorm):
                nn.init.ones_(m.weight)
                nn.init.zeros_(m.bias)
            elif isinstance(m, WindowMSA):
                m.init_weights()

    def load_pretrained(self, checkpoint):
        sd = checkpoint.get("state_dict", checkpoint.get("model", checkpoint)) if isinstance(checkpoint, dict) else checkpoint
        if self.convert_weights:
            sd = swin_converter(sd)
        state = OrderedDict()
        for k, v in sd.items():
            if k.startswith("backbone."):
                state[k[9:]] = v
        if not state:
            state = OrderedDict(sd)
        if state and next(iter(state)).startswith("module."):
            state = OrderedDict((k[7:], v) for k, v in state.items())
        own = self.state_dict()
        for key in [k for k in state if "relative_position_bias_table" in k and k in own]:
            pre, cur = state[key], own[key]
            (L1, nH1), (L2, nH2) = pre.shape, cur.shape
            if nH1 != nH2:
                warnings.warn(f"Error in loading {key}, pass")
                state.pop(key)
            elif L1 != L2:
                S1, S2 = int(L1 ** 0.5), int(L2 ** 0.5)
                r = F.interpolate(pre.permute(1, 0).reshape(1, nH1, S1, S1).float(), size=(S2, S2), mode="bicubic")
                state[key] = r.view(nH2, L2).permute(1, 0).contiguous().to(pre.dtype)
        for key in [k for k in state if k.endswith("relative_position_index") and k in own
                    and tuple(state[k].shape) != tuple(own[k].shape)]:
            state.pop(key)
        return self.load_state_dict(state, strict=False)

    def forward_tokens(self, x):
        x, hw = self.patch_embed(x)
        outs = []
        for i, stage in enumerate(self.stages):
            x, hw, out, out_hw = stage(x, hw)
            if i in self.out_indices:
                n = getattr(self, f"norm{i}")
                outs.append((hip_ops.layer_norm(out, n.weight, n.bias, n.eps), out_hw))
        return outs

    def forward(self, x):
        return [t.view(-1, *hw, t.shape[-1]).permute(0, 3, 1, 2).contiguous() for t, hw in self.forward_tokens(x)]


def swin_converter(ckpt):
    out = OrderedDict()

    def regroup(t, last_dim):
        C4 = t.shape[-1] if last_dim else t.shape[0]
        g = t.reshape(*t.shape[:-1], 4, C4 // 4) if last_dim else t.reshape(4, C4 // 4)
        g = g[..., [0, 2, 1, 3], :] if last_dim else g[[0, 2, 1, 3], :]
        return g.transpose(-1, -2).reshape(t.shape)

    for k, v in ckpt.items():
        if k.startswith("head"):
            continue
        nk, nv = k, v
        if k.startswith("layers"):
            if "attn." in k:
                nk = k.replace("attn.", "attn.w_msa.")
            elif "mlp.fc1." in k:
                nk = k.replace("mlp.fc1.", "ffn.layers.0.0.")
            elif "mlp.fc2." in k:
                nk = k.replace("mlp.fc2.", "ffn.layers.1.")
            elif "mlp." in k:
                nk = k.replace("mlp.", "ffn.")
            elif "downsample" in k:
                if "reduction." in k:
                    nv = regroup(v, last_dim=True)
                elif "norm." in k:
                    nv = regroup(v, last_dim=False)
            nk = nk.replace("layers", "stages", 1)
        elif k.startswith("patch_embed") and "proj" in k:
            nk = k.replace("proj", "projection")
        out["backbone." + nk] = nv
    return out
```

co-detr-tensorrt_amd/csrc/gemm_persist.h:

```cpp
#pragma once
#include <hip/hip_runtime.h>
#include <stdint.h>

#include <type_traits>

#include "codetr_hip.h"
#include "device_prims.h"
#include "gemm_epilogue.h"
#include "large_lds.h"

namespace {

typedef unsigned u32x2v __attribute__((__vector_size__(2 * sizeof(unsigned))));

constexpr int kSlot = 32768;
constexpr int kOpBytes = 16384;
constexpr int kBiasBytes = 32768;

struct PersistArgs {
  const unsigned char* X;
  const unsigned char* W;
  const unsigned short* bias;
  const unsigned short* R;
  unsigned short* Y;
  int M, N, K;
  int tiles_n, T, nk;
  int G;
};

__device__ __forceinline__ int key64(int row) {
  const int q = (row >> 2) & 3;
  return q ^ ((q & 1) << 1);
}

struct RingProducer {
  int h;
  const unsigned char* Wp;
  const unsigned char* Xp;
  unsigned voffW[2], voffX[2];

  __device__ __forceinline__ void set_item(const PersistArgs& a, int wave, int lane, int tile, int kb) {
    const int K = a.K, K2 = K * 2;
    const int tm = tile / a.tiles_n, tn = tile - tm * a.tiles_n;
    const int m0 = tm * 256, n0 = tn * 256;
    const int nmax = a.N - 1 - n0, mmax = a.M - 1 - m0;
    int ln = lane;
    asm volatile("" : "+v"(ln));
#pragma unroll
    for (int q = 0; q < 2; ++q) {
      const int r = (wave + 8 * q) * 16 + (ln >> 2);
      const int rw = (r & 192) + 4 * (r & 15) + ((r >> 4) & 3);
      const unsigned co = (unsigned)((((ln & 3) ^ key64(r)) * 16));
      const int rn = rw < nmax ? rw : nmax, rm = r < mmax ? r : mmax;
      voffW[q] = (unsigned)rn * (unsigned)K2 + co;
      voffX[q] = (unsigned)rm * (unsigned)K2 + co;
    }
    Wp = a.W + ((size_t)n0 * K + (size_t)kb * 64) * 2;
    Xp = a.X + ((size_t)m0 * K + (size_t)kb * 64) * 2;
    h = 2 * kb;
  }

  __device__ __forceinline__ void piece(int g, int slot, unsigned lds0, int wave) const {
    const unsigned dst = lds0 + (unsigned)slot * kSlot + (unsigned)wave * 1024u;
    if (g < 2) lds_dma16(Wp, voffW[g], dst + (unsigned)g * 8192u);
    else lds_dma16(Xp, voffX[g - 2], dst + kOpBytes + (unsigned)(g - 2) * 8192u);
  }

  __device__ __forceinline__ bool step(int ke) {
    ++h;
    if (h >= 2 * ke) return false;
    Wp += 64;
    Xp += 64;
    return true;
  }
};

__device__ __forceinline__ unsigned frag_offset(int op, int row0, int lane) {
  const int fa = lane & 15, fc = lane >> 4;
  return (unsigned)(op + (row0 + fa) * 64 + ((fc ^ key64(fa)) * 16));
}

__device__ __forceinline__ void stage_bias(unsigned char* bias_lds, const unsigned short* bias, int N, int tid) {
  for (int i = tid; i * 8 < N; i += 512)
    *reinterpret_cast<u32x4*>(bias_lds + i * 16) = *reinterpret_cast<const u32x4*>(bias + i * 8);
}

template <class T, int ACT, bool HAS_BIAS, bool HAS_RES>
__device__ __forceinline__ bool tile_epilogue(f32x4 (&acc)[4][8], const PersistArgs& a, int tile, int m_half, int strip,
                                              int lane, const unsigned char* bias_lds) {
  const int fa = lane & 15;
  const int tm = tile / a.tiles_n, tn = tile - tm * a.tiles_n;
  const int m0 = tm * 256 + m_half * 128, n0 = tn * 256 + strip * 64;
  const int g = lane >> 4, nl = 4 * fa;
  const int mleft = a.M - m0, nleft = a.N - n0;
  const unsigned rowb = (unsigned)a.N * 2u;
  const unsigned span = (mleft > 0 && nleft > 0) ? (unsigned)(mleft < 128 ? mleft : 128) * rowb : 0u;
  const unsigned voff = nl < nleft ? (unsigned)(4 * g) * rowb + (unsigned)nl * 2u : 0x80000000u;
  const int mrem = mleft - 4 * g;
  const __amdgpu_buffer_rsrc_t rres = __builtin_amdgcn_make_buffer_rsrc(
      const_cast<unsigned char*>(reinterpret_cast<const unsigned char*>(a.R)) + ((size_t)m0 * a.N + n0) * 2, 0,
      HAS_RES ? span : 0u, 0x00020000);
  uint2 rr[8][4];
  auto load_res = [&](int j0, int j1) {
#pragma unroll
    for (int j = j0; j < j1; ++j)
#pragma unroll
      for (int r = 0; r < 4; ++r) {
        const u32x2v t2 = __builtin_amdgcn_raw_buffer_load_b64(rres, j * 16 + r < mrem ? voff : 0x80000000u,
                                                                 (unsigned)(j * 16 + r) * rowb, 0);
        rr[j][r] = uint2{t2[0], t2[1]};
      }
  };
  const bool stored = a.M > m0 && a.N > n0;
  if (stored) {
    float bias4[4] = {0.f, 0.f, 0.f, 0.f};
    if (HAS_BIAS) {
      const int nb = n0 + nl < a.N ? n0 + nl : 0;
      const uint2 b2 = *reinterpret_cast<const uint2*>(bias_lds + nb * 2);
      bias4[0] = T::to_f32((unsigned short)(b2.x & 0xffffu));
      bias4[1] = T::to_f32((unsigned short)(b2.x >> 16));
      bias4[2] = T::to_f32((unsigned short)(b2.y & 0xffffu));
      bias4[3] = T::to_f32((unsigned short)(b2.y >> 16));
    }
    const __amdgpu_buffer_rsrc_t ry = __builtin_amdgcn_make_buffer_rsrc(
        reinterpret_cast<unsigned char*>(a.Y) + ((size_t)m0 * a.N + n0) * 2, 0, span, 0x00020000);
    if (HAS_RES) load_res(0, 4);
#pragma unroll
    for (int j = 0; j < 8; ++j) {
      if (HAS_RES && j == 2) load_res(4, 8);
#pragma unroll
      for (int r = 0; r < 4; ++r) {
        float x[4];
#pragma unroll
        for (int i = 0; i < 4; ++i) x[i] = acc[i][j][r] + bias4[i];
        const f32x2 x01 = epi_act2<ACT, HAS_RES>(f32x2{x[0], x[1]}), x23 = epi_act2<ACT, HAS_RES>(f32x2{x[2], x[3]});
        uint2 o = {T::pack2(x01.x, x01.y), T::pack2(x23.x, x23.y)};
        if (HAS_RES) {
          const uint2 q = rr[j][r];
          const float y0 = T::to_f32((unsigned short)(o.x & 0xffffu)) + T::to_f32((unsigned short)(q.x & 0xffffu));
          const float y1 = T::to_f32((unsigned short)(o.x >> 16)) + T::to_f32((unsigned short)(q.x >> 16));
          const float y2 = T::to_f32((unsigned short)(o.y & 0xffffu)) + T::to_f32((unsigned short)(q.y & 0xffffu));
          const float y3 = T::to_f32((unsigned short)(o.y >> 16)) + T::to_f32((unsigned short)(q.y >> 16));
          o = uint2{T::pack2(y0, y1), T::pack2(y2, y3)};
        }
        if (!(kAbl & 16))
          __builtin_amdgcn_raw_buffer_store_b64(u32x2v{o.x, o.y}, ry, j * 16 + r < mrem ? voff : 0x80000000u,
                                                (unsigned)(j * 16 + r) * rowb, 0);
      }
    }
  }
  return stored;
}

bool persist_supported(int64_t M, int64_t N, int64_t K) {
  return M > 0 && N > 0 && K >= 128 && K % 64 == 0 && N % 8 == 0 && M <= 0x7fffffffLL && N <= 16384 &&
         255 * K * 2 + 64 < 0x7fffffffLL;
}

int persist_check(const void* X, const void* W, const void* bias, const void* R, const void* Y, const void* ws, int64_t M,
                  int64_t N, int64_t K, int act) {
  if (!X || !W || !Y || M <= 0 || N <= 0 || K <= 0) return CODETR_E_BADARG;
  if (act < 0 || act > 2 || !persist_supported(M, N, K)) return CODETR_E_UNSUPPORTED;
  if ((reinterpret_cast<uintptr_t>(X) | reinterpret_cast<uintptr_t>(W) | reinterpret_cast<uintptr_t>(Y) |
       reinterpret_cast<uintptr_t>(R) | reinterpret_cast<uintptr_t>(bias) | reinterpret_cast<uintptr_t>(ws)) & 15)
    return CODETR_E_BADARG;
  return 0;
}

int persist_grid() { return device_cus() / 8 * 8; }

int persist_fill(PersistArgs& a, const void* X, const void* W, const void* bias, const void* R, void* Y, int64_t M, int64_t N,
                 int64_t K, int G) {
  const int64_t tiles_m = (M + 255) / 256, tiles_n = (N + 255) / 256, T = tiles_m * tiles_n;
  if (T > 0x3fffffff) return CODETR_E_TOO_LARGE;
  if (G <= 0) return CODETR_E_BADARG;
  a.X = static_cast<const unsigned char*>(X);
  a.W = static_cast<const unsigned char*>(W);
  a.bias = static_cast<const unsigned short*>(bias);
  a.R = static_cast<const unsigned short*>(R);
  a.Y = static_cast<unsigned short*>(Y);
  a.M = (int)M; a.N = (int)N; a.K = (int)K;
  a.tiles_n = (int)tiles_n; a.T = (int)T; a.nk = (int)(K / 64);
  a.G = G;
  return 0;
}

template <class Args, class Kernel>
int persist_launch(hipStream_t st, const Args& a, Kernel kernel) {
  void (*k)(const Args);
  if (a.bias && a.R) k = kernel(std::true_type{}, std::true_type{});
  else if (a.bias) k = kernel(std::true_type{}, std::false_type{});
  else if (a.R) k = kernel(std::false_type{}, std::true_type{});
  else k = kernel(std::false_type{}, std::false_type{});
  hipLaunchKernelGGL(k, dim3((unsigned)a.G), dim3(512), 0, st, a);
  const hipError_t err = hipGetLastError();
  return err == hipSuccess ? 0 : (int)err;
}

}
```

co-detr-tensorrt_amd/csrc/gemm_pp.hip:

```cpp

#ifndef CODETR_PP_ABL
#define CODETR_PP_ABL 0
#endif
namespace {
constexpr int kAbl = CODETR_PP_ABL;
}

#include "gemm_persist.h"

namespace {

#ifdef CODETR_PP_STAMPS
__device__ unsigned long long* g_pp_stamps = nullptr;
#define PP_T(i) const unsigned long long pp_t##i = __builtin_readcyclecounter()
#define PP_ACC(k, a, b) pp_acc[k] += pp_t##b - pp_t##a
#define PP_STAMPS_OUT()                                                                    \
  if (lane == 0 && g_pp_stamps) {                                                          \
    pp_acc[7] = __builtin_readcyclecounter() - pp_k0;                                      \
    unsigned long long* o = g_pp_stamps + ((size_t)blockIdx.x * 8 + wave) * 8;             \
    for (int i = 0; i < 8; ++i) o[i] = pp_acc[i];                                          \
  }
#else
#define PP_T(i)
#define PP_ACC(k, a, b)
#define PP_STAMPS_OUT()
#endif

struct PpArgs : PersistArgs {
  int rounds;
  int rem;
};

__device__ __forceinline__ void seg_barrier() {
  __builtin_amdgcn_sched_barrier(0);
  __builtin_amdgcn_s_barrier();
  __builtin_amdgcn_sched_barrier(0);
}

__device__ __forceinline__ int item_tile(const PpArgs& a, int w, int idx) {
  const int D = a.rounds * a.G;
  if (w < a.rem) {
    if (idx == 0) return D + w;
    --idx;
  }
  if (idx >= a.rounds) return -1;
  return (w & 7) * (D >> 3) + idx * (a.G >> 3) + (w >> 3);
}

template <class T, int ACT, bool HAS_BIAS, bool HAS_RES, int NS>
__global__ __launch_bounds__(512) __attribute__((amdgpu_waves_per_eu(2, 2))) void linear_pp_kernel(const PpArgs a) {
  __shared__ __attribute__((aligned(16))) unsigned char lds[NS * kSlot + (HAS_BIAS ? kBiasBytes : 0)];
  using frag = typename T::frag;
  constexpr int PP = 4;
  constexpr int VMN = PP * (NS - 2);

  const int tid = threadIdx.x, lane = tid & 63;
  const int wave = __builtin_amdgcn_readfirstlane(tid >> 6);
  const int grp = wave >> 2, wn = wave & 3;
  const int wg = blockIdx.x;
  const int nh = 2 * a.nk;
  const unsigned lds0 = (unsigned)(uintptr_t)((__attribute__((address_space(3))) unsigned char*)lds);

#ifdef CODETR_PP_STAMPS
  unsigned long long pp_acc[8] = {0, 0, 0, 0, 0, 0, 0, 0};
  const unsigned long long pp_k0 = __builtin_readcyclecounter();
#endif
  int c_idx = 0;
  int c_tile = item_tile(a, wg, 0);
  if (c_tile < 0) return;

  RingProducer prod;
  int p_idx = 0, p_tile = c_tile;
  prod.set_item(a, wave, lane, p_tile, 0);
  auto produce_piece = [&](int g, int slot) { prod.piece(g, slot, lds0, wave); };
  auto produce_advance = [&]() {
    if (p_tile < 0 || prod.step(a.nk)) return;
    p_tile = item_tile(a, wg, ++p_idx);
    if (p_tile >= 0) prod.set_item(a, wave, lane, p_tile, 0);
  };

  const unsigned offA = frag_offset(0, wn * 64, lane), offB = frag_offset(kOpBytes, grp * 128, lane);

  f32x4 acc[4][8];
  frag fw[4], fx[8];

  if (HAS_BIAS) stage_bias(lds + NS * kSlot, a.bias, a.N, tid);
#pragma unroll
  for (int s = 0; s < NS - 1; ++s) {
#pragma unroll
    for (int g = 0; g < PP; ++g) produce_piece(g, s);
    produce_advance();
  }
  wait_vmcnt<VMN>();
  asm volatile("s_waitcnt lgkmcnt(0)" ::: "memory");
  seg_barrier();
  int post = 0;
  int ws = 0;

  auto load_seg = [&]() {
    PP_T(0);
    const unsigned char* rbase = lds + ws * kSlot;
    const int fs = ws == 0 ? NS - 1 : ws - 1;
    if (!(kAbl & 4)) {
#pragma unroll
      for (int i = 0; i < 4; ++i) fw[i] = *reinterpret_cast<const frag*>(rbase + offA + i * 1024);
#pragma unroll
      for (int j = 0; j < 8; ++j) fx[j] = *reinterpret_cast<const frag*>(rbase + offB + j * 1024);
    }
    if (!(kAbl & 1)) {
#pragma unroll
      for (int g = 0; g < PP; ++g) produce_piece(g, fs);
    }
    produce_advance();
    PP_T(1);
    if (post > 0) {
      wait_vmcnt<VMN + 32>();
      --post;
    } else {
      wait_vmcnt<VMN>();
    }
    PP_T(2);
    asm volatile("s_waitcnt lgkmcnt(0)" ::: "memory");
    PP_T(3);
    seg_barrier();
    PP_T(4);
    PP_ACC(0, 0, 1); PP_ACC(1, 1, 2); PP_ACC(2, 2, 3); PP_ACC(3, 3, 4);
  };
  auto mfma_seg = [&](bool firstk) {
    PP_T(5);
    __builtin_amdgcn_s_setprio(1);
#pragma unroll
    for (int i = 0; i < 4; ++i)
#pragma unroll
      for (int j = 0; j < 8; ++j) {
        if (kAbl & 2) asm volatile("" ::"v"(fw[i]), "v"(fx[j]));
        else if (firstk) acc[i][j] = T::mfma(fx[j], fw[i], f32x4{0.f, 0.f, 0.f, 0.f});
        else acc[i][j] = T::mfma(fx[j], fw[i], acc[i][j]);
      }
    __builtin_amdgcn_s_setprio(0);
    PP_T(6);
    seg_barrier();
    PP_T(7);
    PP_ACC(4, 5, 6); PP_ACC(5, 6, 7);
  };

  while (c_tile >= 0) {
    if (grp == 1) seg_barrier();
    load_seg();
    mfma_seg(true);
    ws = ws + 1 == NS ? 0 : ws + 1;
    for (int h = 1; h < nh; ++h) {
      load_seg();
      mfma_seg(false);
      ws = ws + 1 == NS ? 0 : ws + 1;
    }
    if (grp == 0) seg_barrier();

    PP_T(8);
    const bool stored = tile_epilogue<T, ACT, HAS_BIAS, HAS_RES>(acc, a, c_tile, grp, wn, lane, lds + NS * kSlot);
    PP_T(9);
    PP_ACC(6, 8, 9);
    post = stored && !(kAbl & 16) ? NS - 2 : 0;
    c_tile = item_tile(a, wg, ++c_idx);
  }
  wait_vmcnt<0>();
  PP_STAMPS_OUT();
}

template <class T>
int launch_pp(hipStream_t st, const void* X, const void* W, const void* bias, const void* R, void* Y, int64_t M, int64_t N,
              int64_t K, int act, int flags) {
  if (const int rc = persist_check(X, W, bias, R, Y, nullptr, M, N, K, act)) return rc;
  PpArgs a;
  if (const int rc = persist_fill(a, X, W, bias, R, Y, M, N, K, persist_grid())) return rc;
  a.rounds = a.T / a.G;
  a.rem = a.T - a.rounds * a.G;
  if ((int64_t)256 * K * 2 > 0x7fffffffLL) return CODETR_E_TOO_LARGE;
  if (flags != 0) return CODETR_E_UNSUPPORTED;
  switch (act) {
    case 0: return persist_launch(st, a, [](auto hb, auto hr) { return &linear_pp_kernel<T, 0, hb(), hr(), 4>; });
    case 1: return persist_launch(st, a, [](auto hb, auto hr) { return &linear_pp_kernel<T, 1, hb(), hr(), 4>; });
    default: return persist_launch(st, a, [](auto hb, auto hr) { return &linear_pp_kernel<T, 2, hb(), hr(), 4>; });
  }
}

}

extern "C" {

int codetr_linear_pp_supported(int64_t M, int64_t N, int64_t K) { return persist_supported(M, N, K) ? 1 : 0; }

int codetr_linear_pp_preferred(int64_t M, int64_t N, int64_t K, int act, int has_residual) {
  (void)act;
  (void)has_residual;
  if (!persist_supported(M, N, K) || K < 768 || N < 384) return 0;
  const int64_t tn = (N + 255) / 256, tiles = ((M + 255) / 256) * tn;
  return tiles >= 200 && N * 8 >= tn * 256 * 7 ? 1 : 0;
}

int codetr_linear_pp_f16(void* stream, const void* x_dev, const void* w_dev, const void* bias_dev, const void* residual_dev,
                         void* y_dev, int64_t M, int64_t N, int64_t K, int act, int flags) {
  return launch_pp<HalfT>(static_cast<hipStream_t>(stream), x_dev, w_dev, bias_dev, residual_dev, y_dev, M, N, K, act, flags);
}

int codetr_linear_pp_bf16(void* stream, const void* x_dev, const void* w_dev, const void* bias_dev, const void* residual_dev,
                          void* y_dev, int64_t M, int64_t N, int64_t K, int act, int flags) {
#if CODETR_PP_ABL
  return CODETR_E_UNSUPPORTED;
#endif
  return launch_pp<BFloatT>(static_cast<hipStream_t>(stream), x_dev, w_dev, bias_dev, residual_dev, y_dev, M, N, K, act, flags);
}

}
```

runner/codetr_runner.cpp:

```cpp
#include <dlfcn.h>
#include <hip/hip_runtime.h>

#include <algorithm>
#include <chrono>
#include <cstdint>
#include <cstdio>
#include <cstdlib>
#include <cstring>
#include <fstream>
#include <map>
#include <string>
#include <type_traits>
#include <utility>
#include <vector>

#include "codetr_hip.h"

union Arg {
  const void* p;
  long long i;
  float f;
};
struct Entry {
  const char* name;
  int nargs;
  int (*call)(void* fn, const Arg* a);
  const char* kinds;
};

template <class T>
constexpr char kind_of() {
  static_assert(std::is_pointer_v<T> || std::is_same_v<T, float> || (std::is_integral_v<T> && (sizeof(T) == 4 || sizeof(T) == 8)),
                "codetr_hip.h: a launch takes pointers, float and 32- / 64-bit integers only");
  return std::is_pointer_v<T> ? 'p' : std::is_same_v<T, float> ? 'f' : sizeof(T) == 8 ? 'l' : std::is_unsigned_v<T> ? 'u' : 'i';
}
template <class T>
T from_arg(const Arg& a) {
  if constexpr (std::is_pointer_v<T>) return (T)a.p;
  else if constexpr (std::is_floating_point_v<T>) return a.f;
  else return (T)a.i;
}
template <class F>
struct Trampoline;
template <class... A>
struct Trampoline<int(A...)> {
  static constexpr int nargs = sizeof...(A);
  static constexpr char kinds[] = {kind_of<A>()..., '\0'};
  template <size_t... I>
  static int call_at(void* fn, const Arg* a, std::index_sequence<I...>) {
    return reinterpret_cast<int (*)(A...)>(fn)(from_arg<A>(a[I])...);
  }
  static int call(void* fn, const Arg* a) { return call_at(fn, a, std::index_sequence_for<A...>{}); }
};
#define ENTRY(name) {#name, Trampoline<decltype(name)>::nargs, Trampoline<decltype(name)>::call, Trampoline<decltype(name)>::kinds},
#include "dispatch_gen.inc"
static_assert(kPlanAbi == CODETR_HIP_ABI_VERSION, "regenerate: python tools/gen_runner_dispatch.py > runner/dispatch_gen.inc");

#define HIP_OK(expr)                                                                                      \
  do {                                                                                                    \
    hipError_t e_ = (expr);                                                                               \
    if (e_ != hipSuccess) {                                                                               \
      fprintf(stderr, "codetr_runner: %s failed: %s (%s:%d)\n", #expr, hipGetErrorString(e_), __FILE__, __LINE__); \
      exit(2);                                                                                            \
    }                                                                                                     \
  } while (0)

enum Kind : uint8_t { kInt = 0, kFloat = 1, kDev = 2, kNull = 3, kHost = 4, kStream = 5 };
struct PArg {
  uint8_t kind;
  long long i = 0;
  float f = 0.f;
  uint32_t seg = 0;
  uint64_t off = 0;
  std::vector<unsigned char> host;
};
struct Call {
  const Entry* entry;
  void* fn;
  std::vector<PArg> args;
};
struct Io {
  std::string name, dtype;
  uint32_t seg;
  uint64_t off, nbytes;
  std::vector<long long> shape;
};

struct Reader {
  std::ifstream f;
  template <class T>
  T get() {
    T v;
    f.read(reinterpret_cast<char*>(&v), sizeof(T));
    if (!f) {
      fprintf(stderr, "codetr_runner: truncated plan\n");
      exit(2);
    }
    return v;
  }
  void bytes(void* dst, size_t n) {
    f.read(reinterpret_cast<char*>(dst), (std::streamsize)n);
    if (!f) {
      fprintf(stderr, "codetr_runner: truncated plan\n");
      exit(2);
    }
  }
  std::string str(size_t n) {
    std::string s(n, '\0');
    if (n) bytes(&s[0], n);
    return s;
  }
};

static std::vector<unsigned char> read_file(const std::string& path) {
  std::ifstream f(path, std::ios::binary | std::ios::ate);
  if (!f) {
    fprintf(stderr, "codetr_runner: cannot open %s\n", path.c_str());
    exit(2);
  }
  std::vector<unsigned char> b((size_t)f.tellg());
  f.seekg(0);
  f.read(reinterpret_cast<char*>(b.data()), (std::streamsize)b.size());
  return b;
}

int main(int argc, char** argv) {
  std::string plan_path, lib_path = "libcodetr_hip.so", out_dir;
  int iters = 20;
  bool use_graph = true;
  std::map<std::string, std::string> inputs;
  for (int i = 1; i < argc; ++i) {
    const std::string a = argv[i];
    auto next = [&]() -> std::string {
      if (i + 1 >= argc) {
        fprintf(stderr, "codetr_runner: %s needs a value\n", a.c_str());
        exit(2);
      }
      return argv[++i];
    };
    if (a == "--plan") plan_path = next();
    else if (a == "--lib") lib_path = next();
    else if (a == "--iters") iters = atoi(next().c_str());
    else if (a == "--no-graph") use_graph = false;
    else if (a == "--out-dir") out_dir = next();
    else if (a == "--list-entries") {
      for (const Entry& e : kEntries) printf("%s %s\n", e.name, e.kinds);
      return 0;
    }
    else if (a == "--input") {
      const std::string kv = next();
      const size_t eq = kv.find('=');
      if (eq == std::string::npos) {
        fprintf(stderr, "codetr_runner: --input name=file\n");
        return 2;
      }
      inputs[kv.substr(0, eq)] = kv.substr(eq + 1);
    } else {
      fprintf(stderr, "usage: codetr_runner --plan P [--lib L] [--iters N] [--no-graph] [--input name=file] [--out-dir D]\n");
      return 2;
    }
  }
  if (plan_path.empty()) {
    fprintf(stderr, "codetr_runner: --plan is required\n");
    return 2;
  }

  void* lib = dlopen(lib_path.c_str(), RTLD_NOW | RTLD_LOCAL);
  if (!lib) {
    fprintf(stderr, "codetr_runner: cannot load %s: %s\n", lib_path.c_str(), dlerror());
    return 2;
  }
  auto abi = reinterpret_cast<int (*)()>(dlsym(lib, "codetr_hip_abi_version"));
  auto strerr = reinterpret_cast<const char* (*)(int)>(dlsym(lib, "codetr_hip_strerror"));
  if (!abi || !strerr || abi() != kPlanAbi) {
    fprintf(stderr, "codetr_runner: %s has ABI %d, this runner was generated for ABI %d\n", lib_path.c_str(), abi ? abi() : -1, kPlanAbi);
    return 2;
  }

  Reader r;
  r.f.open(plan_path, std::ios::binary);
  if (!r.f) {
    fprintf(stderr, "codetr_runner: cannot open %s\n", plan_path.c_str());
    return 2;
  }
  const std::string magic = r.str(12);
  if (magic != std::string("CODETRPLAN\0\2", 12)) {
    fprintf(stderr, "codetr_runner: %s is not a plan of this format\n", plan_path.c_str());
    return 2;
  }
  const int plan_abi = r.get<int32_t>();
  if (plan_abi != kPlanAbi) {
    fprintf(stderr, "codetr_runner: plan recorded with ABI %d, library / runner have %d: re-export the plan\n", plan_abi, kPlanAbi);
    return 2;
  }
  const uint32_t nseg = r.get<uint32_t>();
  std::vector<uint64_t> seg_size(nseg);
  std::vector<unsigned char*> seg_base(nseg, nullptr);
  uint64_t total = 0;
  for (uint32_t i = 0; i < nseg; ++i) {
    seg_size[i] = r.get<uint64_t>();
    if (seg_size[i]) {
      HIP_OK(hipMalloc(reinterpret_cast<void**>(&seg_base[i]), seg_size[i]));
      total += seg_size[i];
    }
  }
  const uint32_t nblob = r.get<uint32_t>();
  uint64_t uploaded = 0;
  {
    std::vector<unsigned char> buf;
    for (uint32_t i = 0; i < nblob; ++i) {
      const uint32_t seg = r.get<uint32_t>();
      const uint64_t off = r.get<uint64_t>(), n = r.get<uint64_t>();
      if (seg >= nseg || !seg_base[seg] || off > seg_size[seg] || n > seg_size[seg] - off) {
        fprintf(stderr, "codetr_runner: blob %u outside its segment\n", i);
        return 2;
      }
      buf.resize(n);
      if (n) r.bytes(buf.data(), n);
      HIP_OK(hipMemcpy(seg_base[seg] + off, buf.data(), n, hipMemcpyHostToDevice));
      uploaded += n;
    }
  }
  const uint32_t ncall = r.get<uint32_t>();
  std::vector<Call> calls(ncall);
  const size_t nentries = sizeof(kEntries) / sizeof(kEntries[0]);
  for (uint32_t c = 0; c < ncall; ++c) {
    const std::string name = r.str(r.get<uint16_t>());
    const Entry* e = nullptr;
    for (size_t k = 0; k < nentries; ++k)
      if (name == kEntries[k].name) e = &kEntries[k];
    const int nargs = r.get<uint8_t>();
    if (!e || e->nargs != nargs) {
      fprintf(stderr, "codetr_runner: plan calls %s/%d, unknown to this runner\n", name.c_str(), nargs);
      return 2;
    }
    calls[c].entry = e;
    calls[c].fn = dlsym(lib, name.c_str());
    if (!calls[c].fn) {
      fprintf(stderr, "codetr_runner: %s does not export %s\n", lib_path.c_str(), name.c_str());
      return 2;
    }
    calls[c].args.resize(nargs);
    for (int j = 0; j < nargs; ++j) {
      PArg& a = calls[c].args[j];
      a.kind = r.get<uint8_t>();
      switch (a.kind) {
        case kInt: a.i = r.get<int64_t>(); break;
        case kFloat: a.f = r.get<float>(); break;
        case kDev:
          a.seg = r.get<uint32_t>();
          a.off = r.get<uint64_t>();
          if (a.seg >= nseg || !seg_base[a.seg] || a.off >= seg_size[a.seg]) {
            fprintf(stderr, "codetr_runner: call %u (%s) points outside its segment\n", c, name.c_str());
            return 2;
          }
          break;
        case kHost: {
          const uint32_t n = r.get<uint32_t>();
          if (n > (1u << 20)) {
            fprintf(stderr, "codetr_runner: call %u (%s) carries a %u-byte host argument\n", c, name.c_str(), n);
            return 2;
          }
          a.host.resize(n);
          if (n) r.bytes(a.host.data(), n);
          break;
        }
        case kNull:
        case kStream: break;
        default: fprintf(stderr, "codetr_runner: bad argument kind %d\n", a.kind); return 2;
      }
    }
  }
  const uint32_t nio = r.get<uint32_t>();
  std::vector<Io> ios(nio);
  for (auto& io : ios) {
    io.name = r.str(r.get<uint16_t>());
    io.dtype = r.str(r.get<uint16_t>());
    io.seg = r.get<uint32_t>();
    io.off = r.get<uint64_t>();
    io.nbytes = r.get<uint64_t>();
    io.shape.resize(r.get<uint8_t>());
    for (auto& d : io.shape) d = r.get<int64_t>();
    if (io.seg >= nseg || !seg_base[io.seg] || io.off > seg_size[io.seg] || io.nbytes > seg_size[io.seg] - io.off) {
      fprintf(stderr, "codetr_runner: tensor %s lies outside its segment\n", io.name.c_str());
      return 2;
    }
  }

  for (const auto& kv : inputs) {
    const Io* io = nullptr;
    for (const auto& x : ios)
      if (x.name == kv.first) io = &x;
    if (!io) {
      fprintf(stderr, "codetr_runner: the plan has no tensor named %s\n", kv.first.c_str());
      return 2;
    }
    const auto bytes = read_file(kv.second);
    if (bytes.size() != io->nbytes) {
      fprintf(stderr, "codetr_runner: %s holds %zu bytes, %s needs %llu\n", kv.second.c_str(), bytes.size(), io->name.c_str(),
              (unsigned long long)io->nbytes);
      return 2;
    }
    HIP_OK(hipMemcpy(seg_base[io->seg] + io->off, bytes.data(), bytes.size(), hipMemcpyHostToDevice));
  }

  hipStream_t stream;
  HIP_OK(hipStreamCreate(&stream));
  int max_nargs = 0;
  for (const Entry& e : kEntries) max_nargs = std::max(max_nargs, e.nargs);
  std::vector<Arg> av(max_nargs);
  auto replay = [&]() {
    for (const Call& c : calls) {
      for (size_t j = 0; j < c.args.size(); ++j) {
        const PArg& a = c.args[j];
        switch (a.kind) {
          case kInt: av[j].i = a.i; break;
          case kFloat: av[j].i = 0; av[j].f = a.f; break;
          case kDev: av[j].p = seg_base[a.seg] + a.off; break;
          case kHost: av[j].p = a.host.data(); break;
          case kStream: av[j].p = stream; break;
          default: av[j].p = nullptr; break;
        }
      }
      const int rc = c.entry->call(c.fn, av.data());
      if (rc != 0) {
        fprintf(stderr, "codetr_runner: %s failed: %s (code %d)\n", c.entry->name, strerr(rc), rc);
        exit(3);
      }
    }
  };
  replay();
  HIP_OK(hipStreamSynchronize(stream));
  hipGraphExec_t exec = nullptr;
  if (use_graph) {
    hipGraph_t graph;
    HIP_OK(hipStreamBeginCapture(stream, hipStreamCaptureModeThreadLocal));
    replay();
    HIP_OK(hipStreamEndCapture(stream, &graph));
    HIP_OK(hipGraphInstantiate(&exec, graph, nullptr, nullptr, 0));
    HIP_OK(hipGraphLaunch(exec, stream));
    HIP_OK(hipStreamSynchronize(stream));
  }
  std::vector<double> ms;
  for (int it = 0; it < iters; ++it) {
    const auto t0 = std::chrono::high_resolution_clock::now();
    if (exec) HIP_OK(hipGraphLaunch(exec, stream));
    else replay();
    HIP_OK(hipStreamSynchronize(stream));
    ms.push_back(std::chrono::duration<double, std::milli>(std::chrono::high_resolution_clock::now() - t0).count());
  }
  std::sort(ms.begin(), ms.end());

  std::string shapes;
  for (const auto& io : ios) {
    if (io.name == "batch_inputs" || io.name == "img_masks") continue;
    std::vector<unsigned char> host(io.nbytes);
    HIP_OK(hipMemcpy(host.data(), seg_base[io.seg] + io.off, io.nbytes, hipMemcpyDeviceToHost));
    if (!out_dir.empty()) {
      std::ofstream o(out_dir + "/" + io.name + ".bin", std::ios::binary);
      o.write(reinterpret_cast<const char*>(host.data()), (std::streamsize)host.size());
    }
    shapes += (shapes.empty() ? "" : ", ") + std::string("\"") + io.name + "\": {\"dtype\": \"" + io.dtype + "\", \"shape\": [";
    for (size_t d = 0; d < io.shape.size(); ++d) shapes += (d ? ", " : "") + std::to_string(io.shape[d]);
    shapes += "]}";
  }
  printf("{\"launches\": %u, \"segments_bytes\": %llu, \"uploaded_bytes\": %llu, \"hipgraph\": %s, \"iters\": %d, "
         "\"p50_ms\": %.3f, \"min_ms\": %.3f, \"outputs\": {%s}}\n",
         ncall, (unsigned long long)total, (unsigned long long)uploaded, exec ? "true" : "false", iters,
         ms.empty() ? 0.0 : ms[ms.size() / 2], ms.empty() ? 0.0 : ms[0], shapes.c_str());
  return 0;
}
```

runner/dispatch_gen.inc:

```
static const int kPlanAbi = 54;
static const Entry kEntries[] = {
ENTRY(codetr_msda_forward_f16)
ENTRY(codetr_msda_forward_bf16)
ENTRY(codetr_msda_forward_f32)
ENTRY(codetr_msda_forward_f64)
ENTRY(codetr_msda_op4_forward_f16)
ENTRY(codetr_msda_op4_forward_bf16)
ENTRY(codetr_msda_fused_forward_f16)
ENTRY(codetr_msda_fused_forward_bf16)
ENTRY(codetr_msda_fused_forward_ref32_f16)
ENTRY(codetr_msda_fused_forward_ref32_bf16)
ENTRY(codetr_msda_encoder_forward_packed_f16)
ENTRY(codetr_msda_encoder_forward_packed_bf16)
ENTRY(codetr_patch_im2col_b16)
ENTRY(codetr_im2col_tokens_b16)
ENTRY(codetr_conv_tokens_f16)
ENTRY(codetr_conv_tokens_bf16)
ENTRY(codetr_conv_im2col_nchw_b16)
ENTRY(codetr_maxpool_tokens_b16)
ENTRY(codetr_topk_f16)
ENTRY(codetr_topk_bf16)
ENTRY(codetr_topk_chunked_f16)
ENTRY(codetr_topk_chunked_bf16)
ENTRY(codetr_linear_f16)
ENTRY(codetr_linear_bf16)
ENTRY(codetr_linear_bf16_f16out)
ENTRY(codetr_encoder_projections_f16)
ENTRY(codetr_encoder_projections_bf16)
ENTRY(codetr_encoder_projections_posgen_f16)
ENTRY(codetr_encoder_projections_posgen_bf16)
ENTRY(codetr_linear_xadd_f16)
ENTRY(codetr_linear_xadd_bf16)
ENTRY(codetr_linear_ln_f16)
ENTRY(codetr_linear_ln_bf16)
ENTRY(codetr_linear_fp8)
ENTRY(codetr_cast_fp8_f16)
ENTRY(codetr_layernorm_fp8_f16)
ENTRY(codetr_linear_fp8mx)
ENTRY(codetr_cast_fp8mx_f16)
ENTRY(codetr_layernorm_fp8mx_f16)
ENTRY(codetr_window_attention_fp8mx_f16)
ENTRY(codetr_add_f16)
ENTRY(codetr_add_bf16)
ENTRY(codetr_sigmoid_f16)
ENTRY(codetr_sigmoid_bf16)
ENTRY(codetr_gather_rows_b16)
ENTRY(codetr_decode_boxes_f16)
ENTRY(codetr_decode_boxes_bf16)
ENTRY(codetr_valid_ratios_f16)
ENTRY(codetr_valid_ratios_bf16)
ENTRY(codetr_linear_splitk_f16)
ENTRY(codetr_linear_splitk_bf16)
ENTRY(codetr_linear_sk_f16)
ENTRY(codetr_linear_sk_bf16)
ENTRY(codetr_swin_mlp_f16)
ENTRY(codetr_swin_mlp_bf16)
ENTRY(codetr_linear_pp_f16)
ENTRY(codetr_linear_pp_bf16)
ENTRY(codetr_mask_pyramid)
ENTRY(codetr_query_sine_embed_f16)
ENTRY(codetr_query_sine_embed_bf16)
ENTRY(codetr_encoder_geometry_f16)
ENTRY(codetr_encoder_geometry_bf16)
ENTRY(codetr_row_max_f16)
ENTRY(codetr_row_max_bf16)
ENTRY(codetr_preprocess_u8_f16)
ENTRY(codetr_preprocess_u8_f32)
ENTRY(codetr_batched_nms_f32)
ENTRY(codetr_preprocess_batch_u8_f16)
ENTRY(codetr_preprocess_batch_u8_bf16)
ENTRY(codetr_preprocess_batch_u8_f32)
ENTRY(codetr_postprocess_detections_f16)
ENTRY(codetr_postprocess_detections_bf16)
ENTRY(codetr_postprocess_detections_f32)
ENTRY(codetr_postprocess_softnms_f16)
ENTRY(codetr_postprocess_softnms_bf16)
ENTRY(codetr_postprocess_softnms_f32)
ENTRY(codetr_preprocess_views_u8_f16)
ENTRY(codetr_preprocess_views_u8_bf16)
ENTRY(codetr_preprocess_views_u8_f32)
ENTRY(codetr_tta_merge_f16)
ENTRY(codetr_tta_merge_bf16)
ENTRY(codetr_tta_merge_f32)
ENTRY(codetr_preprocess_tiles_u8_f16)
ENTRY(codetr_preprocess_tiles_u8_bf16)
ENTRY(codetr_preprocess_tiles_u8_f32)
ENTRY(codetr_slice_merge_f16)
ENTRY(codetr_slice_merge_bf16)
ENTRY(codetr_slice_merge_f32)
ENTRY(codetr_draw_detections_f16)
ENTRY(codetr_draw_detections_bf16)
ENTRY(codetr_draw_detections_f32)
ENTRY(codetr_frames_to_rgb_u8)
ENTRY(codetr_track_update_f16)
ENTRY(codetr_track_update_bf16)
ENTRY(codetr_track_update_f32)
ENTRY(codetr_msda_backward_f16)
ENTRY(codetr_msda_backward_f32)
ENTRY(codetr_msda_backward_f64)
ENTRY(codetr_layernorm_f16)
ENTRY(codetr_layernorm_bf16)
ENTRY(codetr_patch_merge_layernorm_f16)
ENTRY(codetr_patch_merge_layernorm_bf16)
ENTRY(codetr_window_attention_f16)
ENTRY(codetr_window_attention_bf16)
ENTRY(codetr_window_attention_fp8out_f16)
ENTRY(codetr_window_attention_ex)
ENTRY(codetr_mha_attention_f16)
ENTRY(codetr_mha_attention_bf16)
ENTRY(codetr_decoder_layer_f16)
ENTRY(codetr_decoder_layer_bf16)
ENTRY(codetr_groupnorm_tokens_f16)
ENTRY(codetr_groupnorm_tokens_bf16)
ENTRY(codetr_sine_pos_tokens_f16)
ENTRY(codetr_sine_pos_tokens_bf16)
ENTRY(codetr_ffn_relu_f16)
ENTRY(codetr_ffn_relu_ln_f16)
ENTRY(codetr_ffn_relu_ln2_f16)
ENTRY(codetr_ffn_fp8)
ENTRY(codetr_ffn_relu_ln2_bf16)
ENTRY(codetr_ffn_pack_w2_f16)
ENTRY(codetr_ffn_oproj_relu_ln2_f16)
ENTRY(codetr_ffn_oproj_relu_ln2_bf16)
};
```

Baseline: 96.08.

## Fold Swin LayerNorm into consumer GEMM using producer-epilogue row statistics

Adds a persistent-GEMM epilogue that emits per-64-column partial sum and sum-of-squares for each output row, plus a small finalize kernel that turns them into row mean and rstd. The following GEMM uses weights pre-scaled by gamma and a column-fold vector, so the LayerNorm becomes an epilogue correction instead of a separate normalisation pass. This is applied across Swin blocks for proj->norm2->fc1 and fc2->next norm1->qkv. The aim is to skip a full read and normalisation of the activations per LayerNorm, at the cost of an extra finalize launch, a stats buffer, and numerical differences from computing LN algebraically in fp32 against fp16 folded weights.

```diff
diff --git a/__graft_entry__.py b/__graft_entry__.py
--- a/__graft_entry__.py
+++ b/__graft_entry__.py
@@ -20,7 +20,7 @@
     csrc = os.path.join(PKG_ROOT, "csrc")
     so = os.path.join(PKG_ROOT, "codetr", "libcodetr_hip.so")
     srcs = [os.path.join(csrc, f) for f in os.listdir(csrc) if f.endswith((".hip", ".h", "Makefile"))]
-    srcs += [os.path.join(ROOT, "include", h) for h in ("codetr_hip.h", "codetr_jpeg.h", "codetr_jpeg_dec.h", "codetr_assign.h", "codetr_wbf.h", "codetr_motion.h", "codetr_appearance.h", "codetr_redact.h")]
+    srcs += [os.path.join(ROOT, "include", h) for h in ("codetr_hip.h", "codetr_jpeg.h", "codetr_jpeg_dec.h", "codetr_assign.h", "codetr_wbf.h", "codetr_motion.h", "codetr_appearance.h", "codetr_redact.h", "codetr_lnfold.h")]
     if _newer(so, srcs):
         subprocess.check_call(["make", "-C", csrc, "-s", "-j4"])
     runner_dir = os.path.join(ROOT, "runner")
diff --git a/co-detr-tensorrt_amd/codetr/_kernel_names.py b/co-detr-tensorrt_amd/codetr/_kernel_names.py
--- a/co-detr-tensorrt_amd/codetr/_kernel_names.py
+++ b/co-detr-tensorrt_amd/codetr/_kernel_names.py
@@ -37,6 +37,7 @@
     "linear_pp_kernel",
     "linear_sk_kernel",
     "linear_xs_kernel",
+    "ln_stats_finalize_kernel",
     "maxpool_tokens_kernel",
     "mha_attention_kernel",
     "motion_finish_kernel",
diff --git a/co-detr-tensorrt_amd/codetr/_lnfold.py b/co-detr-tensorrt_amd/codetr/_lnfold.py
--- /dev/null
+++ b/co-detr-tensorrt_amd/codetr/_lnfold.py
@@ -0,0 +1,86 @@
+import os
+
+import torch
+
+from . import _cabi, _cheader
+
+HEADER_PATH = os.path.join(os.path.dirname(_cheader.HEADER_PATH), "codetr_lnfold.h")
+if not os.path.isfile(HEADER_PATH):
+    raise ImportError(f"C ABI header not found at {HEADER_PATH}; the folded-LayerNorm binding is derived from it")
+with open(HEADER_PATH) as _f:
+    functions, defines = _cheader.parse(_f.read())
+
+ABI_VERSION = defines["CODETR_LNFOLD_ABI_VERSION"]
+
+SIGNATURES = {name: (_cabi._CTYPE[_cheader.kind(ret, returned=True)], [_cabi._CTYPE[_cheader.kind(t)] for t, _ in params])
+              for name, (ret, params) in functions.items()}
+LAUNCHES = tuple(name for name, (ret, params) in functions.items() if ret == "int" and params[:1] == [("void *", "stream")])
+
+for _k in ("linear_pp_stats", "linear_pp_lnfold", "ln_stats_finalize"):
+    _cabi.CALLS.setdefault(_k, 0)
+_lib = None
+
+
+def load():
+    global _lib
+    if _lib is not None:
+        return _lib
+    _cabi.load()
+    lib = _cabi._lib
+    for name, (res, args) in SIGNATURES.items():
+        try:
+            fn = getattr(lib, name)
+        except AttributeError as e:
+            raise ImportError(f"{_cabi.LIB_PATH} does not export {name}; rebuild the extension") from e
+        fn.restype = res
+        fn.argtypes = args
+    ver = lib.codetr_lnfold_abi_version()
+    if ver != ABI_VERSION:
+        raise ImportError(f"{_cabi.LIB_PATH} has folded-LayerNorm ABI version {ver}, host expects {ABI_VERSION}; rebuild "
+                          "the extension")
+    _lib = lib
+    return lib
+
+
+def _launch(name, *args):
+    rc = getattr(load(), name)(*args)
+    if _cabi.RECORDER is not None and rc == 0:
+        _cabi.RECORDER.append((name, args))
+    _cabi.check(rc, name)
+
+
+def _sfx(dtype):
+    return "f16" if dtype == torch.float16 else "bf16"
+
+
+def stats_bytes(M, N):
+    return int(load().codetr_lnfold_stats_bytes(M, N))
+
+
+def linear_pp_stats(x2d, weight, bias, residual2d, out2d, stats):
+    _cabi.CALLS["linear"] += 1
+    _cabi.CALLS["linear_pp"] += 1
+    _cabi.CALLS["linear_pp_stats"] += 1
+    M, K = x2d.shape
+    _launch("codetr_linear_pp_stats_" + _sfx(x2d.dtype), _cabi.current_stream_ptr(x2d.device), x2d.data_ptr(),
+            weight.data_ptr(), bias.data_ptr() if bias is not None else None, residual2d.data_ptr(), out2d.data_ptr(),
+            stats.data_ptr(), M, weight.shape[0], K)
+    return out2d
+
+
+def ln_stats_finalize(stats, rowstat, M, N, eps):
+    _cabi.CALLS["ln_stats_finalize"] += 1
+    _launch("codetr_ln_stats_finalize", _cabi.current_stream_ptr(stats.device), stats.data_ptr(), rowstat.data_ptr(), M, N,
+            float(eps))
+    return rowstat
+
+
+def linear_pp_lnfold(x2d, w_folded, colfold, rowstat, act, out2d):
+    _cabi.CALLS["linear"] += 1
+    _cabi.CALLS["linear_pp"] += 1
+    _cabi.CALLS["linear_pp_lnfold"] += 1
+    M, K = x2d.shape
+    _launch("codetr_linear_pp_lnfold_" + _sfx(x2d.dtype), _cabi.current_stream_ptr(x2d.device), x2d.data_ptr(),
+            w_folded.data_ptr(), colfold.data_ptr(), rowstat.data_ptr(), out2d.data_ptr(), M, w_folded.shape[0], K,
+            _cabi._ACT[act])
+    return out2d
diff --git a/co-detr-tensorrt_amd/codetr/export.py b/co-detr-tensorrt_amd/codetr/export.py
--- a/co-detr-tensorrt_amd/codetr/export.py
+++ b/co-detr-tensorrt_amd/codetr/export.py
@@ -3,7 +3,7 @@
 
 import torch
 
-from . import _cabi
+from . import _cabi, _lnfold
 
 MAGIC = b"CODETRPLAN\x00\x02"
 import re
@@ -108,7 +108,7 @@
     used = set()
     enc_calls = []
     for name, args in calls:
-        argtypes = _cabi.SIGNATURES[name][1]
+        argtypes = (_cabi.SIGNATURES.get(name) or _lnfold.SIGNATURES[name])[1]
         enc = []
         for j, (a, t) in enumerate(zip(args, argtypes)):
             if j == 0:
diff --git a/co-detr-tensorrt_amd/codetr/hip_ops.py b/co-detr-tensorrt_amd/codetr/hip_ops.py
--- a/co-detr-tensorrt_amd/codetr/hip_ops.py
+++ b/co-detr-tensorrt_amd/codetr/hip_ops.py
@@ -7,7 +7,7 @@
 import torch
 import torch.nn.functional as F
 
-from . import _appearance, _assign, _cabi, _jpeg, _jpeg_dec, _motion, _redact, _wbf
+from . import _appearance, _assign, _cabi, _jpeg, _jpeg_dec, _lnfold, _motion, _redact, _wbf
 
 NATIVE = {"msda", "linear(f16/bf16, K%64==0)", "layer_norm(f16/bf16)", "swin_window_attention(f16, head_dim 32)",
           "msda_fused(softmax + sampling locations in-kernel)", "groupnorm_tokens(f16, 8 ch/group)",
@@ -166,6 +166,72 @@
         if ok:
             return out.view(*x.shape[:-1], N)
     return linear(layer_norm(x, norm_weight, norm_bias, eps), weight, bias, act=act)
+
+
+LN_FOLD_PP = True
+
+
+def ln_fold_supported(x, w_producer, norm_weight, norm_bias, w_consumer, act):
+    if not (LN_FOLD_PP and LINEAR_PP and x.is_cuda and x.dtype in (torch.float16, torch.bfloat16)
+            and not torch.is_grad_enabled() and act in (None, "gelu") and norm_weight is not None and norm_bias is not None):
+        return False
+    C = x.shape[-1]
+    M = x.numel() // max(C, 1)
+    if not (w_producer.shape[0] == C == w_consumer.shape[1] == norm_weight.shape[0] and w_producer.shape[1] % 64 == 0
+            and all(t.dtype == x.dtype for t in (w_producer, norm_weight, norm_bias, w_consumer))):
+        return False
+    return (M > 0 and _cabi.linear_splitk_plan(M, C, w_producer.shape[1])[0] == 1
+            and _cabi.linear_splitk_plan(M, w_consumer.shape[0], C)[0] == 1
+            and _cabi.linear_pp_preferred(M, C, w_producer.shape[1], None, True)
+            and _cabi.linear_pp_preferred(M, w_consumer.shape[0], C, act, False))
+
+
+def linear_stats(x, weight, bias, residual):
+    _gpu(x, "linear_stats")
+    K, N = x.shape[-1], weight.shape[0]
+    x2 = x.reshape(-1, K)
+    x2 = x2 if x2.is_contiguous() else x2.contiguous()
+    w = weight if weight.is_contiguous() else weight.contiguous()
+    r2 = residual.reshape(-1, N)
+    r2 = r2 if r2.is_contiguous() else r2.contiguous()
+    M = x2.shape[0]
+    out = torch.empty((M, N), dtype=x.dtype, device=x.device)
+    if not (M > 0 and _cabi.linear_supported(x, weight) and _persistent_ok(None, None, out, x2, w, r2, bias)
+            and _cabi.linear_splitk_plan(M, N, K)[0] == 1 and _cabi.linear_pp_preferred(M, N, K, None, True)):
+        return linear(x, weight, bias, residual=residual), None
+    stats = torch.empty((M, (N + 63) // 64, 2), dtype=torch.float32, device=x.device)
+    with torch.cuda.device(x.device):
+        _timed_linear(lambda: _lnfold.linear_pp_stats(x2, w, bias, r2, out, stats), x.device, M, N, K)
+    return out.view(*residual.shape[:-1], N), stats
+
+
+def _lnfold_weights(weight, bias, norm_weight, norm_bias):
+    def build():
+        W = weight.detach().double()
+        wf = (W * norm_weight.detach().double()[None, :]).to(weight.dtype).contiguous()
+        bp = W @ norm_bias.detach().double()
+        if bias is not None:
+            bp = bp + bias.detach().double()
+        return wf, torch.stack([wf.double().sum(1), bp]).float().contiguous()
+
+    return derived([weight, norm_weight, norm_bias] + ([bias] if bias is not None else []), "_codetr_lnfold", build)
+
+
+def linear_lnfold(x, stats, norm_weight, norm_bias, eps, weight, bias=None, act=None):
+    _gpu(x, "linear_lnfold")
+    K, N = x.shape[-1], weight.shape[0]
+    x2 = x.reshape(-1, K)
+    x2 = x2 if x2.is_contiguous() else x2.contiguous()
+    M = x2.shape[0]
+    wf, colfold = _lnfold_weights(weight, bias, norm_weight, norm_bias)
+    out = torch.empty((M, N), dtype=x.dtype, device=x.device)
+    if stats is None or M < 2 or not _persistent_ok(None, None, out, x2, wf, None, None):
+        return linear(layer_norm(x, norm_weight, norm_bias, eps), weight, bias, act=act)
+    rowstat = torch.empty(((M + 1) // 2 * 2, 2), dtype=torch.float32, device=x.device)
+    with torch.cuda.device(x.device):
+        _lnfold.ln_stats_finalize(stats, rowstat, M, K, eps)
+        _timed_linear(lambda: _lnfold.linear_pp_lnfold(x2, wf, colfold, rowstat, act, out), x.device, M, N, K)
+    return out.view(*x.shape[:-1], N)
 
 
 XADD = True
@@ -1727,7 +1793,7 @@
 MSDA_FP32_REF = True
 
 
-_SWITCH_DEFAULTS = {"ENC_POSGEN": True, "WINDOW_BIAS_LANE": True, "LINEAR_PP": True, "SWIN_MLP": True, "SWIN_MLP_MIN_ROWS": 32768, "LN_GEMM": True, "XADD": True, "XADD_MIN_ROWS": 0, "MERGE_LN": True, "MSDA_ENCODER": True,
+_SWITCH_DEFAULTS = {"ENC_POSGEN": True, "WINDOW_BIAS_LANE": True, "LINEAR_PP": True, "LN_FOLD_PP": True, "SWIN_MLP": True, "SWIN_MLP_MIN_ROWS": 32768, "LN_GEMM": True, "XADD": True, "XADD_MIN_ROWS": 0, "MERGE_LN": True, "MSDA_ENCODER": True,
                     "MSDA_FP32_REF": True, "FP8_MIN_TILES": 96,
                     "R50_NATIVE": True, "R50_CONV_IM2COL": False}
 
diff --git a/co-detr-tensorrt_amd/codetr/swin.py b/co-detr-tensorrt_amd/codetr/swin.py
--- a/co-detr-tensorrt_amd/codetr/swin.py
+++ b/co-detr-tensorrt_amd/codetr/swin.py
@@ -160,7 +160,7 @@
     def takes_norm(self, query, hw_shape):
         return hip_ops.swin_window_attention_supported(query, self.w_msa.embed_dims, self.w_msa.num_heads, self.window_size)
 
-    def forward(self, query, hw_shape, identity=None, pre_norm=None):
+    def forward(self, query, hw_shape, identity=None, pre_norm=None, in_stats=None, out_stats=False):
         B, L, C = query.shape
         H, W = hw_shape
         if L != H * W:
@@ -168,12 +168,18 @@
         ws, sh = self.window_size, self.shift_size
         m = self.w_msa
         if hip_ops.swin_window_attention_supported(query, C, m.num_heads, ws):
-            if pre_norm is not None:
+            if in_stats is not None:
+                qkv = hip_ops.linear_lnfold(query, in_stats, pre_norm[0], pre_norm[1], pre_norm[2], m.qkv.weight, m.qkv.bias)
+            elif pre_norm is not None:
                 qkv = hip_ops.linear_ln(query, pre_norm[0], pre_norm[1], pre_norm[2], m.qkv.weight, m.qkv.bias)
             else:
                 qkv = hip_ops.linear(query, m.qkv.weight, m.qkv.bias)
             o = hip_ops.swin_window_attention(qkv, m.qkv.bias, m.relative_position_bias(), hw_shape, m.num_heads, ws, sh)
+            if out_stats:
+                return hip_ops.linear_stats(o, m.proj.weight, m.proj.bias, identity)
             return hip_ops.linear(o, m.proj.weight, m.proj.bias, residual=identity)
+        if in_stats is not None or out_stats:
+            raise AssertionError("the folded LayerNorm exists on the fused window-attention path only")
         x = query.view(B, H, W, C)
         pad_r, pad_b = (-W) % ws, (-H) % ws
         if pad_r or pad_b:
@@ -207,35 +213,58 @@
                        act_cfg=act_cfg, add_identity=True)
 
     def forward(self, x, hw_shape):
+        return self.forward_stats(x, hw_shape)[0]
+
+    def _folds(self, x, hw_shape):
+        return (hip_ops.LN_FOLD_PP and getattr(self, "fp8_mode", None) is None and isinstance(self.norm1, nn.LayerNorm)
+                and isinstance(self.norm2, nn.LayerNorm) and self.ffn.add_identity and x.is_cuda
+                and self.attn.takes_norm(x, hw_shape))
+
+    def forward_stats(self, x, hw_shape, in_stats=None, next_block=None):
         n1, n2 = self.norm1, self.norm2
         mode = getattr(self, "fp8_mode", None)
         if mode is not None and x.is_cuda and x.dtype == torch.float16 and self.attn.takes_norm(x, hw_shape):
             rows = x.shape[0] * x.shape[1]
             if mode == "calibrate":
-                return self._forward_fp8_calibrate(x, hw_shape)
+                return self._forward_fp8_calibrate(x, hw_shape), None
             if mode == "run" and all(hip_ops.linear_fp8_supported(rows, w) for w in self._fp8_weights()):
-                return self._forward_fp8(x, hw_shape)
+                return self._forward_fp8(x, hw_shape), None
             if mode == "mx":
                 ops = getattr(self, "fp8_ops", None) or ("qkv", "proj", "fc1", "fc2")
                 ws = dict(zip(("qkv", "proj", "fc1", "fc2"), self._fp8_weights()))
                 if ops and all(hip_ops.linear_fp8_supported(rows, ws[o]) for o in ops):
-                    return self._forward_fp8mx(x, hw_shape)
-        if (isinstance(n1, nn.LayerNorm) and self.attn.takes_norm(x, hw_shape)
+                    return self._forward_fp8mx(x, hw_shape), None
+        m = self.attn.w_msa
+        fc1, fc2 = self.ffn.layers[0][0], self.ffn.layers[1]
+        folds = self._folds(x, hw_shape)
+        fold2 = folds and hip_ops.ln_fold_supported(x, m.proj.weight, n2.weight, n2.bias, fc1.weight, self.ffn.act)
+        st2 = None
+        if folds and in_stats is not None:
+            x = self.attn(x, hw_shape, identity=x, pre_norm=(n1.weight, n1.bias, n1.eps), in_stats=in_stats, out_stats=fold2)
+        elif (isinstance(n1, nn.LayerNorm) and self.attn.takes_norm(x, hw_shape)
                 and hip_ops.linear_ln_supported(x, n1.weight, self.attn.w_msa.qkv.weight)):
-            x = self.attn(x, hw_shape, identity=x, pre_norm=(n1.weight, n1.bias, n1.eps))
+            x = self.attn(x, hw_shape, identity=x, pre_norm=(n1.weight, n1.bias, n1.eps), out_stats=fold2)
         else:
             h = hip_ops.layer_norm(x, n1.weight, n1.bias, n1.eps)
-            x = self.attn(h, hw_shape, identity=x)
-        fc1, fc2 = self.ffn.layers[0][0], self.ffn.layers[1]
+            x = self.attn(h, hw_shape, identity=x, out_stats=fold2)
+        if fold2:
+            x, st2 = x
+            nb = next_block
+            fold_next = (nb is not None and nb._folds(x, hw_shape)
+                         and hip_ops.ln_fold_supported(x, fc2.weight, nb.norm1.weight, nb.norm1.bias, nb.attn.w_msa.qkv.weight, None))
+            h = hip_ops.linear_lnfold(x, st2, n2.weight, n2.bias, n2.eps, fc1.weight, fc1.bias, act=self.ffn.act)
+            if fold_next:
+                return hip_ops.linear_stats(h, fc2.weight, fc2.bias, x)
+            return hip_ops.linear(h, fc2.weight, fc2.bias, residual=x), None
         if (isinstance(n2, nn.LayerNorm) and self.ffn.add_identity and fc1.bias is not None and fc2.bias is not None
                 and hip_ops.swin_mlp_supported(x, n2.weight, fc1.weight, fc2.weight, self.ffn.act)):
-            return hip_ops.swin_mlp(x, n2.weight, n2.bias, n2.eps, fc1.weight, fc1.bias, fc2.weight, fc2.bias)
+            return hip_ops.swin_mlp(x, n2.weight, n2.bias, n2.eps, fc1.weight, fc1.bias, fc2.weight, fc2.bias), None
         if (isinstance(n2, nn.LayerNorm) and self.ffn.add_identity
                 and hip_ops.linear_ln_supported(x, n2.weight, fc1.weight)):
             h = hip_ops.linear_ln(x, n2.weight, n2.bias, n2.eps, fc1.weight, fc1.bias, act=self.ffn.act)
-            return hip_ops.linear(h, fc2.weight, fc2.bias, residual=x)
+            return hip_ops.linear(h, fc2.weight, fc2.bias, residual=x), None
         h = hip_ops.layer_norm(x, n2.weight, n2.bias, n2.eps)
-        return self.ffn(h, identity=x)
+        return self.ffn(h, identity=x), None
 
 
     def _fp8_weights(self):
@@ -327,8 +356,9 @@
         self.downsample = downsample
 
     def forward(self, x, hw_shape):
-        for blk in self.blocks:
-            x = blk(x, hw_shape)
+        stats = None
+        for i, blk in enumerate(self.blocks):
+            x, stats = blk.forward_stats(x, hw_shape, stats, self.blocks[i + 1] if i + 1 < len(self.blocks) else None)
         if self.downsample is not None:
             x_down, down_hw = self.downsample(x, hw_shape)
             return x_down, down_hw, x, hw_shape
diff --git a/co-detr-tensorrt_amd/csrc/gemm_persist.h b/co-detr-tensorrt_amd/csrc/gemm_persist.h
--- a/co-detr-tensorrt_amd/csrc/gemm_persist.h
+++ b/co-detr-tensorrt_amd/csrc/gemm_persist.h
@@ -85,9 +85,47 @@
     *reinterpret_cast<u32x4*>(bias_lds + i * 16) = *reinterpret_cast<const u32x4*>(bias + i * 8);
 }
 
-template <class T, int ACT, bool HAS_BIAS, bool HAS_RES>
+constexpr int kLnNone = 0, kLnStats = 1, kLnFold = 2;
+constexpr int kFoldBytes = 4096;
+struct LnArgs {
+  float* stats;
+  const float* rowstat;
+  const float* colfold;
+};
+
+template <int LN>
+constexpr int epilogue_stores() {
+  return LN == kLnStats ? 40 : 32;
+}
+
+__device__ __forceinline__ void fold_stage(const PersistArgs& a, const LnArgs& ln, int tile, int wave, int lane, unsigned lds_dst) {
+  if (wave > 3) return;
+  const int tm = tile / a.tiles_n, tn = tile - tm * a.tiles_n;
+  if (wave < 2) {
+    const int left = ((a.M + 1) & ~1) - tm * 256 - 2;
+    const int r = wave * 128 + 2 * lane;
+    lds_dma16(reinterpret_cast<const unsigned char*>(ln.rowstat + (size_t)tm * 512), (unsigned)(r < left ? r : left) * 8u,
+              lds_dst + (unsigned)wave * 1024u);
+  } else {
+    const int left = a.N - tn * 256 - 4;
+    const int c = 4 * lane;
+    lds_dma16(reinterpret_cast<const unsigned char*>(ln.colfold + (wave == 3 ? (size_t)a.N : 0) + (size_t)tn * 256),
+              (unsigned)(c < left ? c : left) * 4u, lds_dst + (unsigned)wave * 1024u);
+  }
+}
+
+__device__ __forceinline__ float row16_sum(float v) {
+  v += dpp_f<kXor1>(v);
+  v += dpp_f<kXor2>(v);
+  v += dpp_f<0x141>(v);
+  v += dpp_f<0x140>(v);
+  return v;
+}
+
+template <class T, int ACT, bool HAS_BIAS, bool HAS_RES, int LN = kLnNone>
 __device__ __forceinline__ bool tile_epilogue(f32x4 (&acc)[4][8], const PersistArgs& a, int tile, int m_half, int strip,
-                                              int lane, const unsigned char* bias_lds) {
+                                              int lane, const unsigned char* bias_lds, const LnArgs* ln = nullptr) {
+  static_assert(LN != kLnFold || (!HAS_BIAS && !HAS_RES), "the folded form carries its bias in colfold and adds no residual");
   const int fa = lane & 15;
   const int tm = tile / a.tiles_n, tn = tile - tm * a.tiles_n;
   const int m0 = tm * 256 + m_half * 128, n0 = tn * 256 + strip * 64;
@@ -112,6 +150,14 @@
       }
   };
   const bool stored = a.M > m0 && a.N > n0;
+  const unsigned rows_here = (unsigned)(mleft < 128 ? mleft : 128);
+  auto load_stat = [&](int j0, int j1) {
+#pragma unroll
+    for (int j = j0; j < j1; ++j)
+#pragma unroll
+      for (int r = 0; r < 4; ++r)
+        rr[j][r] = *reinterpret_cast<const uint2*>(bias_lds + (m_half * 128 + j * 16 + 4 * g + r) * 8);
+  };
   if (stored) {
     float bias4[4] = {0.f, 0.f, 0.f, 0.f};
     if (HAS_BIAS) {
@@ -125,14 +171,40 @@
     const __amdgpu_buffer_rsrc_t ry = __builtin_amdgcn_make_buffer_rsrc(
         reinterpret_cast<unsigned char*>(a.Y) + ((size_t)m0 * a.N + n0) * 2, 0, span, 0x00020000);
     if (HAS_RES) load_res(0, 4);
+    float s4[4] = {0.f, 0.f, 0.f, 0.f};
+    if (LN == kLnFold) {
+      const u32x4 sv = *reinterpret_cast<const u32x4*>(bias_lds + 2048 + (strip * 64 + nl) * 4);
+      const u32x4 bv = *reinterpret_cast<const u32x4*>(bias_lds + 3072 + (strip * 64 + nl) * 4);
+      load_stat(0, 4);
+#pragma unroll
+      for (int i = 0; i < 4; ++i) {
+        s4[i] = __uint_as_float(sv[i]);
+        bias4[i] = __uint_as_float(bv[i]);
+      }
+    }
+    const bool col_ok = nl < nleft;
+    const float inv_cnt = 1.0f / (float)(nleft < 64 ? nleft : 64);
+    const unsigned S8 = (unsigned)((a.N + 63) >> 6) * 8u;
+    const __amdgpu_buffer_rsrc_t rpart = __builtin_amdgcn_make_buffer_rsrc(
+        LN == kLnStats ? ln->stats + ((size_t)m0 * (S8 >> 3) + (size_t)(n0 >> 6)) * 2 : nullptr, 0,
+        LN == kLnStats ? (rows_here - 1u) * S8 + 8u : 0u, 0x00020000);
 #pragma unroll
     for (int j = 0; j < 8; ++j) {
       if (HAS_RES && j == 2) load_res(4, 8);
+      if (LN == kLnFold && j == 2) load_stat(4, 8);
+      float st_mean = 0.f, st_m2 = 0.f;
 #pragma unroll
       for (int r = 0; r < 4; ++r) {
         float x[4];
 #pragma unroll
-        for (int i = 0; i < 4; ++i) x[i] = acc[i][j][r] + bias4[i];
+        for (int i = 0; i < 4; ++i) {
+          if (LN == kLnFold) {
+            const float mu = __uint_as_float(rr[j][r].x), rs = __uint_as_float(rr[j][r].y);
+            x[i] = fmaf(rs, fmaf(-mu, s4[i], acc[i][j][r]), bias4[i]);
+          } else {
+            x[i] = acc[i][j][r] + bias4[i];
+          }
+        }
         const f32x2 x01 = epi_act2<ACT, HAS_RES>(f32x2{x[0], x[1]}), x23 = epi_act2<ACT, HAS_RES>(f32x2{x[2], x[3]});
         uint2 o = {T::pack2(x01.x, x01.y), T::pack2(x23.x, x23.y)};
         if (HAS_RES) {
@@ -146,7 +218,27 @@
         if (!(kAbl & 16))
           __builtin_amdgcn_raw_buffer_store_b64(u32x2v{o.x, o.y}, ry, j * 16 + r < mrem ? voff : 0x80000000u,
                                                 (unsigned)(j * 16 + r) * rowb, 0);
+        if (LN == kLnStats) {
+          float v[4] = {T::to_f32((unsigned short)(o.x & 0xffffu)), T::to_f32((unsigned short)(o.x >> 16)),
+                        T::to_f32((unsigned short)(o.y & 0xffffu)), T::to_f32((unsigned short)(o.y >> 16))};
+          const float mean = row16_sum(col_ok ? (v[0] + v[1]) + (v[2] + v[3]) : 0.f) * inv_cnt;
+          float q = 0.f;
+#pragma unroll
+          for (int i = 0; i < 4; ++i) {
+            const float d = v[i] - mean;
+            q = fmaf(d, d, q);
+          }
+          const float m2 = row16_sum(col_ok ? q : 0.f);
+          if (fa == r) {
+            st_mean = mean;
+            st_m2 = m2;
+          }
+        }
       }
+      if (LN == kLnStats && !(kAbl & 16))
+        __builtin_amdgcn_raw_buffer_store_b64(u32x2v{__float_as_uint(st_mean), __float_as_uint(st_m2)}, rpart,
+                                              fa < 4 && j * 16 + fa < mrem ? (unsigned)(4 * g + fa) * S8 : 0x80000000u,
+                                              (unsigned)(j * 16) * S8, 0);
     }
   }
   return stored;
diff --git a/co-detr-tensorrt_amd/csrc/gemm_pp.hip b/co-detr-tensorrt_amd/csrc/gemm_pp.hip
--- a/co-detr-tensorrt_amd/csrc/gemm_pp.hip
+++ b/co-detr-tensorrt_amd/csrc/gemm_pp.hip
@@ -6,6 +6,7 @@
 constexpr int kAbl = CODETR_PP_ABL;
 }
 
+#include "codetr_lnfold.h"
 #include "gemm_persist.h"
 
 namespace {
@@ -29,6 +30,7 @@
 struct PpArgs : PersistArgs {
   int rounds;
   int rem;
+  LnArgs ln;
 };
 
 __device__ __forceinline__ void seg_barrier() {
@@ -47,12 +49,14 @@
   return (w & 7) * (D >> 3) + idx * (a.G >> 3) + (w >> 3);
 }
 
-template <class T, int ACT, bool HAS_BIAS, bool HAS_RES, int NS>
+template <class T, int ACT, bool HAS_BIAS, bool HAS_RES, int NS, int LN = kLnNone>
 __global__ __launch_bounds__(512) __attribute__((amdgpu_waves_per_eu(2, 2))) void linear_pp_kernel(const PpArgs a) {
-  __shared__ __attribute__((aligned(16))) unsigned char lds[NS * kSlot + (HAS_BIAS ? kBiasBytes : 0)];
+  __shared__ __attribute__((aligned(16))) unsigned char lds[NS * kSlot + (HAS_BIAS ? kBiasBytes : LN == kLnFold ? 2 * kFoldBytes : 0)];
   using frag = typename T::frag;
   constexpr int PP = 4;
   constexpr int VMN = PP * (NS - 2);
+  constexpr int EST = epilogue_stores<LN>();
+  static_assert(VMN + EST <= 63, "vmcnt is a 6-bit counter");
 
   const int tid = threadIdx.x, lane = tid & 63;
   const int wave = __builtin_amdgcn_readfirstlane(tid >> 6);
@@ -85,6 +89,7 @@
   frag fw[4], fx[8];
 
   if (HAS_BIAS) stage_bias(lds + NS * kSlot, a.bias, a.N, tid);
+  if (LN == kLnFold) fold_stage(a, a.ln, c_tile, wave, lane, lds0 + NS * kSlot);
 #pragma unroll
   for (int s = 0; s < NS - 1; ++s) {
 #pragma unroll
@@ -114,7 +119,7 @@
     produce_advance();
     PP_T(1);
     if (post > 0) {
-      wait_vmcnt<VMN + 32>();
+      wait_vmcnt<VMN + EST>();
       --post;
     } else {
       wait_vmcnt<VMN>();
@@ -157,25 +162,86 @@
     if (grp == 0) seg_barrier();
 
     PP_T(8);
-    const bool stored = tile_epilogue<T, ACT, HAS_BIAS, HAS_RES>(acc, a, c_tile, grp, wn, lane, lds + NS * kSlot);
+    const int n_tile = item_tile(a, wg, c_idx + 1);
+    if (LN == kLnFold && n_tile >= 0) fold_stage(a, a.ln, n_tile, wave, lane, lds0 + NS * kSlot + ((c_idx + 1) & 1) * kFoldBytes);
+    const bool stored = tile_epilogue<T, ACT, HAS_BIAS, HAS_RES, LN>(
+        acc, a, c_tile, grp, wn, lane, lds + NS * kSlot + (LN == kLnFold ? (c_idx & 1) * kFoldBytes : 0), &a.ln);
     PP_T(9);
     PP_ACC(6, 8, 9);
     post = stored && !(kAbl & 16) ? NS - 2 : 0;
-    c_tile = item_tile(a, wg, ++c_idx);
+    c_tile = n_tile;
+    ++c_idx;
   }
   wait_vmcnt<0>();
   PP_STAMPS_OUT();
+}
+
+__global__ __launch_bounds__(256) void ln_stats_finalize_kernel(const float2* __restrict__ stats, float2* __restrict__ rowstat,
+                                                                int64_t M, int N, float eps) {
+  const int64_t row = (int64_t)blockIdx.x * 256 + threadIdx.x;
+  if (row >= M) return;
+  const int S = (N + 63) >> 6;
+  const float2* p = stats + row * S;
+  double n = 0.0, mean = 0.0, m2 = 0.0;
+  for (int s = 0; s < S; ++s) {
+    const float2 v = p[s];
+    const double nb = (double)(N - 64 * s < 64 ? N - 64 * s : 64), nn = n + nb;
+    const double d = (double)v.x - mean;
+    mean += d * (nb / nn);
+    m2 += (double)v.y + d * d * (n * nb / nn);
+    n = nn;
+  }
+  rowstat[row] = float2{(float)mean, (float)(1.0 / sqrt(m2 / n + (double)eps))};
+}
+
+template <class T>
+int fill_pp(PpArgs& a, const void* X, const void* W, const void* bias, const void* R, void* Y, int64_t M, int64_t N, int64_t K,
+            int act) {
+  if (const int rc = persist_check(X, W, bias, R, Y, nullptr, M, N, K, act)) return rc;
+  if (const int rc = persist_fill(a, X, W, bias, R, Y, M, N, K, persist_grid())) return rc;
+  a.rounds = a.T / a.G;
+  a.rem = a.T - a.rounds * a.G;
+  a.ln = LnArgs{nullptr, nullptr, nullptr};
+  if ((int64_t)256 * K * 2 > 0x7fffffffLL) return CODETR_E_TOO_LARGE;
+  return 0;
+}
+
+int launch_one(hipStream_t st, const PpArgs& a, void (*k)(const PpArgs)) {
+  hipLaunchKernelGGL(k, dim3((unsigned)a.G), dim3(512), 0, st, a);
+  const hipError_t err = hipGetLastError();
+  return err == hipSuccess ? 0 : (int)err;
+}
+
+template <class T>
+int launch_pp_stats(hipStream_t st, const void* X, const void* W, const void* bias, const void* R, void* Y, void* stats,
+                    int64_t M, int64_t N, int64_t K) {
+  if (!R || !stats || (reinterpret_cast<uintptr_t>(stats) & 15)) return CODETR_E_BADARG;
+  PpArgs a;
+  if (const int rc = fill_pp<T>(a, X, W, bias, R, Y, M, N, K, 0)) return rc;
+  if ((M + 255) / 256 * 256 * ((N + 63) / 64) * 8 > 0x7fffffffLL) return CODETR_E_TOO_LARGE;
+  a.ln.stats = static_cast<float*>(stats);
+  return launch_one(st, a, bias ? &linear_pp_kernel<T, 0, true, true, 4, kLnStats> : &linear_pp_kernel<T, 0, false, true, 4, kLnStats>);
+}
+
+template <class T>
+int launch_pp_fold(hipStream_t st, const void* X, const void* W, const void* colfold, const void* rowstat, void* Y, int64_t M,
+                   int64_t N, int64_t K, int act) {
+  if (!colfold || !rowstat || ((reinterpret_cast<uintptr_t>(colfold) | reinterpret_cast<uintptr_t>(rowstat)) & 15))
+    return CODETR_E_BADARG;
+  if (M < 2) return CODETR_E_UNSUPPORTED;
+  if (act != 0 && act != 2) return CODETR_E_UNSUPPORTED;
+  PpArgs a;
+  if (const int rc = fill_pp<T>(a, X, W, nullptr, nullptr, Y, M, N, K, act)) return rc;
+  a.ln.rowstat = static_cast<const float*>(rowstat);
+  a.ln.colfold = static_cast<const float*>(colfold);
+  return launch_one(st, a, act == 0 ? &linear_pp_kernel<T, 0, false, false, 4, kLnFold> : &linear_pp_kernel<T, 2, false, false, 4, kLnFold>);
 }
 
 template <class T>
 int launch_pp(hipStream_t st, const void* X, const void* W, const void* bias, const void* R, void* Y, int64_t M, int64_t N,
               int64_t K, int act, int flags) {
-  if (const int rc = persist_check(X, W, bias, R, Y, nullptr, M, N, K, act)) return rc;
   PpArgs a;
-  if (const int rc = persist_fill(a, X, W, bias, R, Y, M, N, K, persist_grid())) return rc;
-  a.rounds = a.T / a.G;
-  a.rem = a.T - a.rounds * a.G;
-  if ((int64_t)256 * K * 2 > 0x7fffffffLL) return CODETR_E_TOO_LARGE;
+  if (const int rc = fill_pp<T>(a, X, W, bias, R, Y, M, N, K, act)) return rc;
   if (flags != 0) return CODETR_E_UNSUPPORTED;
   switch (act) {
     case 0: return persist_launch(st, a, [](auto hb, auto hr) { return &linear_pp_kernel<T, 0, hb(), hr(), 4>; });
@@ -211,4 +277,43 @@
   return launch_pp<BFloatT>(static_cast<hipStream_t>(stream), x_dev, w_dev, bias_dev, residual_dev, y_dev, M, N, K, act, flags);
 }
 
-}
+int codetr_lnfold_abi_version(void) { return CODETR_LNFOLD_ABI_VERSION; }
+
+int64_t codetr_lnfold_stats_bytes(int64_t M, int64_t N) { return M <= 0 || N <= 0 ? 0 : M * ((N + 63) / 64) * 8; }
+
+int codetr_linear_pp_stats_f16(void* stream, const void* x_dev, const void* w_dev, const void* bias_dev, const void* residual_dev,
+                               void* y_dev, void* stats_dev, int64_t M, int64_t N, int64_t K) {
+  return launch_pp_stats<HalfT>(static_cast<hipStream_t>(stream), x_dev, w_dev, bias_dev, residual_dev, y_dev, stats_dev, M, N, K);
+}
+
+int codetr_linear_pp_stats_bf16(void* stream, const void* x_dev, const void* w_dev, const void* bias_dev, const void* residual_dev,
+                                void* y_dev, void* stats_dev, int64_t M, int64_t N, int64_t K) {
+#if CODETR_PP_ABL
+  return CODETR_E_UNSUPPORTED;
+#endif
+  return launch_pp_stats<BFloatT>(static_cast<hipStream_t>(stream), x_dev, w_dev, bias_dev, residual_dev, y_dev, stats_dev, M, N, K);
+}
+
+int codetr_ln_stats_finalize(void* stream, const void* stats_dev, void* rowstat_dev, int64_t M, int64_t N, float eps) {
+  if (!stats_dev || !rowstat_dev || M <= 0 || N <= 0) return CODETR_E_BADARG;
+  if (N > 16384 || (M + 255) / 256 > 0x7fffffffLL) return CODETR_E_UNSUPPORTED;
+  hipLaunchKernelGGL(ln_stats_finalize_kernel, dim3((unsigned)((M + 255) / 256)), dim3(256), 0, static_cast<hipStream_t>(stream),
+                     static_cast<const float2*>(stats_dev), static_cast<float2*>(rowstat_dev), M, (int)N, eps);
+  const hipError_t err = hipGetLastError();
+  return err == hipSuccess ? 0 : (int)err;
+}
+
+int codetr_linear_pp_lnfold_f16(void* stream, const void* x_dev, const void* w_dev, const void* colfold_dev,
+                                const void* rowstat_dev, void* y_dev, int64_t M, int64_t N, int64_t K, int act) {
+  return launch_pp_fold<HalfT>(static_cast<hipStream_t>(stream), x_dev, w_dev, colfold_dev, rowstat_dev, y_dev, M, N, K, act);
+}
+
+int codetr_linear_pp_lnfold_bf16(void* stream, const void* x_dev, const void* w_dev, const void* colfold_dev,
+                                 const void* rowstat_dev, void* y_dev, int64_t M, int64_t N, int64_t K, int act) {
+#if CODETR_PP_ABL
+  return CODETR_E_UNSUPPORTED;
+#endif
+  return launch_pp_fold<BFloatT>(static_cast<hipStream_t>(stream), x_dev, w_dev, colfold_dev, rowstat_dev, y_dev, M, N, K, act);
+}
+
+}
diff --git a/include/codetr_lnfold.h b/include/codetr_lnfold.h
--- /dev/null
+++ b/include/codetr_lnfold.h
@@ -0,0 +1,27 @@
+#ifndef CODETR_LNFOLD_H
+#define CODETR_LNFOLD_H
+
+#include <stdint.h>
+
+#ifdef __cplusplus
+extern "C" {
+#endif
+
+#define CODETR_LNFOLD_ABI_VERSION 1
+int codetr_lnfold_abi_version(void);
+int64_t codetr_lnfold_stats_bytes(int64_t M, int64_t N);
+int codetr_linear_pp_stats_f16(void *stream, const void *x_dev, const void *w_dev, const void *bias_dev,
+                               const void *residual_dev, void *y_dev, void *stats_dev, int64_t M, int64_t N, int64_t K);
+int codetr_linear_pp_stats_bf16(void *stream, const void *x_dev, const void *w_dev, const void *bias_dev,
+                                const void *residual_dev, void *y_dev, void *stats_dev, int64_t M, int64_t N, int64_t K);
+int codetr_ln_stats_finalize(void *stream, const void *stats_dev, void *rowstat_dev, int64_t M, int64_t N, float eps);
+int codetr_linear_pp_lnfold_f16(void *stream, const void *x_dev, const void *w_dev, const void *colfold_dev,
+                                const void *rowstat_dev, void *y_dev, int64_t M, int64_t N, int64_t K, int act);
+int codetr_linear_pp_lnfold_bf16(void *stream, const void *x_dev, const void *w_dev, const void *colfold_dev,
+                                 const void *rowstat_dev, void *y_dev, int64_t M, int64_t N, int64_t K, int act);
+
+#ifdef __cplusplus
+}
+#endif
+
+#endif
diff --git a/runner/codetr_runner.cpp b/runner/codetr_runner.cpp
--- a/runner/codetr_runner.cpp
+++ b/runner/codetr_runner.cpp
@@ -15,6 +15,7 @@
 #include <vector>
 
 #include "codetr_hip.h"
+#include "codetr_lnfold.h"
 
 union Arg {
   const void* p;
@@ -55,6 +56,7 @@
 #define ENTRY(name) {#name, Trampoline<decltype(name)>::nargs, Trampoline<decltype(name)>::call, Trampoline<decltype(name)>::kinds},
 #include "dispatch_gen.inc"
 static_assert(kPlanAbi == CODETR_HIP_ABI_VERSION, "regenerate: python tools/gen_runner_dispatch.py > runner/dispatch_gen.inc");
+static_assert(kLnfoldAbi == CODETR_LNFOLD_ABI_VERSION, "regenerate: python tools/gen_runner_dispatch.py > runner/dispatch_gen.inc");
 
 #define HIP_OK(expr)                                                                                      \
   do {                                                                                                    \
@@ -176,6 +178,12 @@
     fprintf(stderr, "codetr_runner: %s has ABI %d, this runner was generated for ABI %d\n", lib_path.c_str(), abi ? abi() : -1, kPlanAbi);
     return 2;
   }
+  auto abi_ln = reinterpret_cast<int (*)()>(dlsym(lib, "codetr_lnfold_abi_version"));
+  if (!abi_ln || abi_ln() != kLnfoldAbi) {
+    fprintf(stderr, "codetr_runner: %s has folded-LayerNorm ABI %d, this runner was generated for %d\n", lib_path.c_str(),
+            abi_ln ? abi_ln() : -1, kLnfoldAbi);
+    return 2;
+  }
 
   Reader r;
   r.f.open(plan_path, std::ios::binary);
@@ -229,6 +237,8 @@
     const Entry* e = nullptr;
     for (size_t k = 0; k < nentries; ++k)
       if (name == kEntries[k].name) e = &kEntries[k];
+    for (const Entry& ce : kLnfoldEntries)
+      if (name == ce.name) e = &ce;
     const int nargs = r.get<uint8_t>();
     if (!e || e->nargs != nargs) {
       fprintf(stderr, "codetr_runner: plan calls %s/%d, unknown to this runner\n", name.c_str(), nargs);
@@ -308,6 +318,7 @@
   HIP_OK(hipStreamCreate(&stream));
   int max_nargs = 0;
   for (const Entry& e : kEntries) max_nargs = std::max(max_nargs, e.nargs);
+  for (const Entry& e : kLnfoldEntries) max_nargs = std::max(max_nargs, e.nargs);
   std::vector<Arg> av(max_nargs);
   auto replay = [&]() {
     for (const Call& c : calls) {
diff --git a/runner/dispatch_gen.inc b/runner/dispatch_gen.inc
--- a/runner/dispatch_gen.inc
+++ b/runner/dispatch_gen.inc
@@ -123,3 +123,11 @@
 ENTRY(codetr_ffn_oproj_relu_ln2_f16)
 ENTRY(codetr_ffn_oproj_relu_ln2_bf16)
 };
+static const int kLnfoldAbi = 1;
+static const Entry kLnfoldEntries[] = {
+ENTRY(codetr_linear_pp_stats_f16)
+ENTRY(codetr_linear_pp_stats_bf16)
+ENTRY(codetr_ln_stats_finalize)
+ENTRY(codetr_linear_pp_lnfold_f16)
+ENTRY(codetr_linear_pp_lnfold_bf16)
+};
```

New measurement: 96.54 (median of 6 runs). About the same (+0.5%).
